# giuliojiang/pbrt-v3-IILE

Measured on AMD Instinct MI355X. Metric: Mray/s on killeroo-simple 1080p (path integrator, rays = Scene::Intersect + IntersectP calls), higher is better.
Workload: dtype f32

## Files before the change

include/iile_gpu.h:

```cpp
#ifndef IILE_GPU_H
#define IILE_GPU_H

#include "iile_scene.h"

#ifdef __cplusplus
extern "C" {
#endif

typedef struct iile_scene iile_scene;

enum {
    IILE_OK = 0,
    IILE_ERR_ARG = 1,
    IILE_ERR_NO_DEVICE = 2,
    IILE_ERR_HIP = 3,
    IILE_ERR_UNSUPPORTED = 4,
    IILE_ERR_TIMEOUT = 5
};

typedef struct iile_render_params {
    int32_t k_begin, k_end;
    int32_t tile_rank, tile_nranks;
    int32_t spp_per_pass;
    int32_t collect_stats;
    int32_t time_kernels;
    int32_t film_on_device;
    void *stream;
} iile_render_params;

typedef struct iile_stats {
    uint64_t camera_rays, closest_rays, shadow_rays;
    uint64_t nodes_closest, nodes_any, tri_tests, tri_hits;
    uint64_t sphere_tests;
    uint64_t nee_evals, zero_radiance;
    uint64_t path_length[8];
    double ms_total;
    double ms_generate, ms_extend, ms_shade, ms_connect, ms_film;
    int32_t n_extend_launches, n_connect_launches , n_shade_launches, n_passes;
    uint64_t n_paths;
    uint64_t workspace_bytes;
    uint64_t ext_rays, ext_nodes, ext_tri_tests, ext_sphere_tests;
    uint64_t any_tri_tests;
    double ms_shadow, ms_mis, ms_resolve;
    uint64_t mis_rays_traced;
    uint64_t ext_rays_traced;
} iile_stats;

int iile_device_count(void);
const char *iile_last_error(void);

int iile_device_select(int32_t device);
int iile_device_alloc(uint64_t bytes, void **out_dev);
void iile_device_free(void *dev);
int iile_device_download(void *dst_host, const void *src_dev, uint64_t bytes, void *stream);
int iile_device_upload(void *dst_dev, const void *src_host, uint64_t bytes, void *stream);
int iile_device_zero(void *dev, uint64_t bytes, void *stream);
int iile_stream_create(void **out_stream);
int iile_stream_wait(void *stream);
void iile_stream_destroy(void *stream);

int iile_scene_create(const iile_scene_desc *desc, iile_scene **out);
void iile_scene_destroy(iile_scene *scene);

int iile_render(iile_scene *scene, const iile_render_params *params, float *film_xyzw, iile_stats *stats);
int iile_render_status(iile_scene *scene, void *stream);
int iile_test_patch_capacity(iile_scene *scene, uint32_t capacity);

int iile_trace_closest(iile_scene *scene, int32_t n, const float *o3, const float *d3, const float *tmax,
                       int32_t *prim, float *tb, iile_stats *stats);
#define IILE_SHAPE_HIT_FLOATS 28
int iile_shape_hit_attributes(iile_scene *scene, int32_t n, const float *o3, const float *d3, const int32_t *prim, float *out);
int iile_trace_any(iile_scene *scene, int32_t n, const float *o3, const float *d3, const float *tmax,
                   int32_t *hit, iile_stats *stats);
int iile_halton_samples(iile_scene *scene, int32_t n, const int32_t *px, const int32_t *py, const int32_t *k,
                        int32_t dim0, int32_t ndims, float *out, uint32_t *index_out);
int iile_camera_rays(iile_scene *scene, int32_t n, const float *pfilm2, const float *plens2, float *o3, float *d3);
int iile_li_samples(iile_scene *scene, int32_t n, const int32_t *px, const int32_t *py, const int32_t *k,
                    float *L3, int32_t *nrays2);
int iile_bsdf_eval(iile_scene *scene, int32_t n, int32_t mat, const float *wo3, const float *wi3, float *out4);
int iile_bsdf_sample(iile_scene *scene, int32_t n, int32_t mat, const float *wo3, const float *u2, float *out7);
int iile_bsdf_eval_ng(iile_scene *scene, int32_t n, int32_t mat, const float *ng3, const float *wo3, const float *wi3, float *out4);
int iile_bsdf_sample_ng(iile_scene *scene, int32_t n, int32_t mat, const float *ng3, const float *wo3, const float *u2, float *out7);
int iile_bsdf_sample_specular(iile_scene *scene, int32_t n, int32_t mat, const float *wo3, const float *u2, float *out9);
int iile_render_probes(iile_scene *scene, int32_t n_probes, const float *pos3, const float *dir3, float *intensity_rgb,
                       float *normals_xyz, float *distance, int32_t outputs_on_device, iile_stats *stats, void *stream);
typedef struct iile_probe_ref_params {
    int32_t max_depth;
    int32_t first_sample;
    int32_t n_samples;
    int32_t spp_total;
    int32_t outputs_on_device;
    void *stream;
} iile_probe_ref_params;
int iile_render_probes_reference(iile_scene *scene, int32_t n_probes, const float *pos3, const float *dir3, const iile_probe_ref_params *params,
                                 float *intensity_rgb, float *weight_sum, float *normals_xyz, float *distance, iile_stats *stats);
int iile_test_probe_ref_group(iile_scene *scene, uint32_t samples_per_group);
int iile_reference_points(iile_scene *scene, int32_t n, const float *pfilm2, uint8_t *valid, float *pos3, float *dir3);
typedef struct iile_direct_params {
    int32_t n_passes, first_pass;
    int32_t accumulate;
    int32_t film_on_device;
    void *stream;
} iile_direct_params;
int iile_render_direct(iile_scene *scene, const iile_direct_params *params, double *film_rgbw);
int iile_iispt_hemi_points(iile_scene *scene, const iile_iispt_task *task, uint8_t *valid, float *pos3, float *dir3);
int iile_iispt_gather(iile_scene *scene, const iile_iispt_task *task, const uint8_t *valid, const float *pos3, const float *dir3,
                      const float *nn_films, int32_t nn_on_device, float *out_rgbw, int32_t out_on_device);
int iile_iispt_hemi_points_batch(iile_scene *scene, const iile_iispt_task *tasks, int32_t n_tasks, uint8_t *valid, float *pos3, float *dir3,
                                 void *stream);
int iile_iispt_gather_batch(iile_scene *scene, const iile_iispt_task *tasks, int32_t n_tasks, const uint8_t *valid, const float *pos3,
                            const float *dir3, const float *nn_films, int32_t nn_on_device, float *out_rgbw, int32_t out_on_device, void *stream);
int iile_iispt_film_add(iile_scene *scene, const iile_iispt_task *tasks, int32_t n_tasks, const float *out_rgbw_dev, double *film_rgbw_dev,
                        int32_t film_w, int32_t film_h, void *stream);
int iile_iispt_film_merge(const double *direct_rgbw_dev, const double *indirect_rgbw_dev, int64_t n_pixels, float *rgb_dev, void *stream);
typedef struct iile_iispt_net iile_iispt_net;
typedef struct iile_iispt_net_weights {
    const float *conv_weight[15], *conv_bias[15];
    const float *bn_weight[5], *bn_bias[5], *bn_mean[5], *bn_var[5];
    float bn_eps;
} iile_iispt_net_weights;
int iile_iispt_net_create(const iile_iispt_net_weights *weights, iile_iispt_net **out);
int iile_iispt_net_load(const char *path, iile_iispt_net **out);
int iile_iispt_net_forward(iile_iispt_net *net, const float *in_dev, float *out_dev, int32_t n, int32_t max_batch, void *stream,
                           float *layer_out_dev, int32_t layer);
int iile_iispt_net_predict(iile_iispt_net *net, const float *intensity_dev, const float *normals_dev, const float *distance_dev,
                           float *pred_dev, const int32_t *slot_of_probe_dev, int32_t n, int32_t film_rows, int32_t max_batch, void *stream);
void iile_iispt_net_destroy(iile_iispt_net *net);
typedef struct iile_bvh_build_stats {
    float ms_total, ms_morton, ms_sort, ms_treelets, ms_upper, ms_flatten, ms_download;
    int32_t n_treelets, n_nodes, n_interior, n_leaf;
} iile_bvh_build_stats;
int iile_bvh_build_hlbvh(int32_t n_prims, const float *bounds6, int32_t max_prims_in_node, iile_bvh_node *nodes_out,
                         int32_t *n_nodes_out, int32_t *order_out, iile_bvh_build_stats *stats);
int iile_bvh_pack_probe(int32_t n_nodes, const iile_bvh_node *nodes, int32_t n_interior, float *wide16, float *wide4_32,
                        int32_t *nested);
int32_t iile_wide_ref_shift(void);
void iile_traversal_limits(int32_t *out3);
int iile_light_sample_li(iile_scene *scene, int32_t light, int32_t n, const float *p3, float *out7);
int iile_light_sample_at(iile_scene *scene, int32_t light, int32_t n, const float *ref_p3, const float *ref_n3, const float *u2, float *out13);
int iile_light_pdf_at(iile_scene *scene, int32_t light, int32_t n, const float *ref_p3, const float *ref_n3, const float *wi3, float *out_pdf);
int iile_light_le(iile_scene *scene, int32_t light, int32_t n, const float *d3, float *out3);
int iile_light_choose(iile_scene *scene, int32_t n, const float *p3, const float *u, int32_t *out_light, float *out_pdf, void *stream);
int iile_texture_eval(iile_scene *scene, int32_t tex, int32_t n, const float *uv2, const float *duv4, float *rgb3);
int iile_texture_eval_p(iile_scene *scene, int32_t tex, int32_t n, const float *uv2, const float *duv4, const float *pdp9, float *rgb3);
int iile_trig_probe(int32_t n, const float *x, float *out3);

#ifdef __cplusplus
}
#endif
#endif
```

pbrt-v3-iile_amd/binding.py:

```python
import ctypes
import os

import numpy as np

_HERE = os.path.dirname(os.path.abspath(__file__))
LIB_DIR = os.path.join(_HERE, "lib")
REPO_ROOT = os.path.dirname(_HERE)
DEFAULT_SCENE = os.path.join(REPO_ROOT, "scenes", "killeroo-simple.pbrt")

c_i32, c_u32, c_u64, c_f32, c_f64 = (ctypes.c_int32, ctypes.c_uint32, ctypes.c_uint64, ctypes.c_float,
                                     ctypes.c_double)
c_vp = ctypes.c_void_p


class HostOverrides(ctypes.Structure):
    _fields_ = [("xres", c_i32), ("yres", c_i32), ("spp", c_i32), ("max_depth", c_i32), ("sampler", c_i32),
                ("accel_split", c_i32), ("bvh_build", c_vp), ("quick_render", c_i32)]


SAMPLERS = {None: 0, "": 0, "halton": 1, "sobol": 2}
SPLITS = {None: 0, "": 0, "sah": 1, "hlbvh": 2, "middle": 3, "equal": 4}


class HostSceneInfo(ctypes.Structure):
# ... 91 lines not shown


class _Sobol(ctypes.Structure):
    _fields_ = [("enabled", c_i32), ("spp", c_i32), ("resolution", c_i32), ("log2_resolution", c_i32), ("n_dims", c_i32),
                ("matrices32", c_vp), ("vdc", c_u32 * 32), ("vdc_inv", c_u32 * 32)]


class SceneDesc(ctypes.Structure):
    _fields_ = SceneDescHead._fields_ + [
        ("tri_n", c_vp), ("tri_uv", c_vp), ("prim_alpha", c_vp), ("n_spheres", c_i32), ("spheres", c_vp), ("n_materials", c_i32),
        ("materials", c_vp), ("n_lights", c_i32), ("lights", c_vp), ("n_env_dist", ctypes.c_int64), ("env_dist", c_vp),
        ("n_textures", c_i32), ("textures", c_vp), ("n_texels", ctypes.c_int64), ("texels", c_vp), ("ewa_lut", c_f32 * 128),
        ("film_filter_wide", c_i32), ("film_filter_table", c_f32 * 256), ("camera", Camera), ("film", FilmDesc), ("halton", _Halton),
        ("integrator", Integrator), ("probe", _ProbeSetup), ("sobol", _Sobol), ("n_quadrics", c_i32), ("quadrics", c_vp),
        ("light_power_all", c_vp)]


MAX_LIGHTS = 8


class Quadric(ctypes.Structure):
    _fields_ = [("o2w", c_f32 * 16), ("o2w_inv", c_f32 * 16), ("kind", c_i32), ("radius", c_f32), ("inner_radius", c_f32),
                ("height", c_f32), ("zmin", c_f32), ("zmax", c_f32), ("phi_max", c_f32), ("reverse_orientation", c_i32),
                ("swaps_handedness", c_i32)]


class Material(ctypes.Structure):
    _fields_ = [("type", c_i32), ("kd", c_f32 * 3), ("ks", c_f32 * 3), ("sigma", c_f32), ("roughness", c_f32), ("alpha", c_f32),
                ("remap_roughness", c_i32), ("eta", c_f32), ("kr", c_f32 * 3), ("kt", c_f32 * 3), ("on_a", c_f32), ("on_b", c_f32),
                ("kd_tex", c_i32), ("ks_tex", c_i32), ("kr_tex", c_i32), ("kt_tex", c_i32), ("bump_tex", c_i32), ("rough_tex", c_i32),
                ("sigma_tex", c_i32), ("opacity", c_f32 * 3), ("roughness_v", c_f32), ("alpha_v", c_f32), ("opacity_tex", c_i32),
                ("rough_tex_v", c_i32), ("cond_eta", c_f32 * 3), ("cond_k", c_f32 * 3)]


MAT_MATTE, MAT_PLASTIC, MAT_UBER, MAT_MIRROR, MAT_GLASS, MAT_METAL, MAT_SUBSTRATE = range(7)
MAT_TRANSLUCENT = 8
QUADRIC_DISK, QUADRIC_CYLINDER = 0, 1
PRIM_SPHERE, PRIM_FLIP, PRIM_QUADRIC = 1, 8, 32
LIGHT_AREA_QUADRIC = 6


class GpuStats(ctypes.Structure):
    _fields_ = [(n, c_u64) for n in ("camera_rays closest_rays shadow_rays nodes_closest nodes_any tri_tests "
                                     "tri_hits sphere_tests nee_evals zero_radiance").split()] + [
        ("path_length", c_u64 * 8),
        ("ms_total", c_f64), ("ms_generate", c_f64), ("ms_extend", c_f64), ("ms_shade", c_f64),
        ("ms_connect", c_f64), ("ms_film", c_f64),
        ("n_extend_launches", c_i32), ("n_connect_launches", c_i32), ("n_shade_launches", c_i32),
        ("n_passes", c_i32), ("n_paths", c_u64), ("workspace_bytes", c_u64),
        ("ext_rays", c_u64), ("ext_nodes", c_u64), ("ext_tri_tests", c_u64), ("ext_sphere_tests", c_u64),
        ("any_tri_tests", c_u64), ("ms_shadow", c_f64), ("ms_mis", c_f64), ("ms_resolve", c_f64),
        ("mis_rays_traced", c_u64), ("ext_rays_traced", c_u64)]

    def as_dict(self):
        d = {}
        for name, _ in self._fields_:
            v = getattr(self, name)
            d[name] = list(v) if name == "path_length" else v
        return d


HOST_SYMBOLS = ["iile_host_load_pbrt", "iile_host_scene_desc", "iile_host_scene_film", "iile_host_scene_get_info",
                "iile_host_scene_free", "iile_host_film_to_rgb", "iile_host_write_pfm", "iile_host_last_error", "iile_host_read_image",
                "iile_host_scene_texture", "iile_host_scene_texture_level", "iile_host_scene_filter_table",
                "iile_host_sobol_matrices", "iile_host_sobol_vdc", "iile_host_write_exr", "iile_host_write_image",
                "iile_host_scene_film_filename", "iile_host_scene_light", "iile_host_scene_quadric_count", "iile_host_scene_quadric",
                "iile_host_scene_material", "iile_host_scene_camera"]
class NetWeights(ctypes.Structure):
    _fields_ = [("conv_weight", c_vp * 15), ("conv_bias", c_vp * 15), ("bn_weight", c_vp * 5), ("bn_bias", c_vp * 5),
                ("bn_mean", c_vp * 5), ("bn_var", c_vp * 5), ("bn_eps", c_f32)]


class ProbeRefParams(ctypes.Structure):
    _fields_ = [("max_depth", c_i32), ("first_sample", c_i32), ("n_samples", c_i32), ("spp_total", c_i32), ("outputs_on_device", c_i32),
                ("stream", c_vp)]


class DirectParams(ctypes.Structure):
    _fields_ = [("n_passes", ctypes.c_int32), ("first_pass", ctypes.c_int32), ("accumulate", ctypes.c_int32), ("film_on_device", ctypes.c_int32),
                ("stream", ctypes.c_void_p)]


GPU_SYMBOLS = ["iile_device_count", "iile_last_error", "iile_scene_create", "iile_scene_destroy", "iile_render",
               "iile_trace_closest", "iile_trace_any", "iile_shape_hit_attributes", "iile_halton_samples", "iile_camera_rays", "iile_li_samples",
               "iile_bsdf_eval", "iile_bsdf_sample", "iile_bsdf_eval_ng", "iile_bsdf_sample_ng", "iile_bsdf_sample_specular", "iile_trig_probe", "iile_texture_eval", "iile_texture_eval_p", "iile_light_sample_li", "iile_light_sample_at", "iile_light_pdf_at", "iile_light_le", "iile_light_choose", "iile_render_probes",
               "iile_render_probes_reference", "iile_test_probe_ref_group", "iile_reference_points",
               "iile_device_select", "iile_device_alloc", "iile_device_free", "iile_device_download", "iile_device_upload", "iile_device_zero",
               "iile_stream_create", "iile_stream_wait", "iile_stream_destroy",
               "iile_iispt_film_add", "iile_iispt_film_merge",
               "iile_iispt_hemi_points", "iile_iispt_gather", "iile_iispt_hemi_points_batch", "iile_iispt_gather_batch", "iile_bvh_build_hlbvh", "iile_bvh_pack_probe", "iile_render_direct",
               "iile_wide_ref_shift", "iile_traversal_limits", "iile_render_status", "iile_test_patch_capacity", "iile_iispt_net_create", "iile_iispt_net_load", "iile_iispt_net_forward", "iile_iispt_net_predict", "iile_iispt_net_destroy"]
DIST_SYMBOLS = ["iile_dist_unique_id", "iile_dist_create", "iile_dist_create_deadline", "iile_dist_abort", "iile_dist_wait", "iile_dist_destroy", "iile_dist_rank", "iile_dist_size", "iile_dist_ranks_seen",
                "iile_dist_film_reduce", "iile_dist_monitor_reduce", "iile_dist_barrier", "iile_dist_sum_u64", "iile_dist_max_f64",
                "iile_dist_rendezvous_file", "iile_dist_rendezvous_file_token", "iile_dist_rendezvous_done", "iile_dist_all_ok",
                "iile_dist_last_error"]
DIST_ID_BYTES = 128

_host = None
_gpu = None
_dist = None


def host_lib():
    global _host
    if _host is None:
        path = os.path.join(LIB_DIR, "libiile_host.so")
        if not os.path.exists(path):
            raise RuntimeError(f"{path} is missing: run __graft_entry__.build() (make -C pbrt-v3-iile_amd/csrc host)")
        lib = ctypes.CDLL(path)
        lib.iile_host_last_error.restype = ctypes.c_char_p
        lib.iile_host_load_pbrt.argtypes = [ctypes.c_char_p, ctypes.POINTER(HostOverrides), ctypes.POINTER(c_vp)]
        lib.iile_host_scene_desc.restype = c_vp
        lib.iile_host_scene_desc.argtypes = [c_vp]
        lib.iile_host_scene_film.restype = ctypes.POINTER(FilmDesc)
        lib.iile_host_scene_film.argtypes = [c_vp]
        lib.iile_host_scene_get_info.argtypes = [c_vp, ctypes.POINTER(HostSceneInfo)]
        lib.iile_host_scene_free.argtypes = [c_vp]
        lib.iile_host_scene_free.restype = None
        lib.iile_host_scene_quadric_count.argtypes = [c_vp]
        lib.iile_host_scene_quadric_count.restype = c_i32
        lib.iile_host_scene_quadric.argtypes = [c_vp, c_i32, ctypes.POINTER(Quadric)]
        lib.iile_host_scene_material.argtypes = [c_vp, c_i32, ctypes.POINTER(Material)]
        lib.iile_host_scene_camera.argtypes = [c_vp, ctypes.POINTER(Camera)]
        lib.iile_host_film_to_rgb.argtypes = [ctypes.POINTER(FilmDesc), c_vp, c_vp]
        lib.iile_host_write_pfm.argtypes = [ctypes.c_char_p, c_vp, c_i32, c_i32]
        lib.iile_host_read_image.argtypes = [ctypes.c_char_p, ctypes.POINTER(c_i32), ctypes.POINTER(c_i32), c_vp]
        lib.iile_host_write_exr.argtypes = [ctypes.c_char_p, c_vp, c_i32, c_i32, c_i32, c_i32, c_i32, c_i32]
        lib.iile_host_write_image.argtypes = [ctypes.c_char_p, ctypes.POINTER(FilmDesc), c_vp]
        lib.iile_host_scene_film_filename.argtypes = [c_vp]
        lib.iile_host_scene_film_filename.restype = ctypes.c_char_p
        lib.iile_host_scene_texture.argtypes = [c_vp, c_i32, ctypes.POINTER(Texture)]
        lib.iile_host_scene_texture_level.argtypes = [c_vp, c_i32, c_i32, c_vp]
        lib.iile_host_scene_filter_table.argtypes = [c_vp, c_vp]
        lib.iile_host_sobol_matrices.argtypes = [c_i32, c_vp, c_vp]
        lib.iile_host_sobol_vdc.argtypes = [c_i32, c_vp, c_vp]
        _host = lib
    return _host


def sobol_matrices(n_dims):
    m32 = np.zeros((n_dims, 52), np.uint32)
    m64 = np.zeros((n_dims, 52), np.uint64)
    if host_lib().iile_host_sobol_matrices(int(n_dims), m32.ctypes.data, m64.ctypes.data) != 0:
        raise RuntimeError(host_lib().iile_host_last_error().decode())
    return m32, m64


def sobol_vdc(log2_resolution):
    vdc = np.zeros(52, np.uint64)
    inv = np.zeros(52, np.uint64)
    if host_lib().iile_host_sobol_vdc(int(log2_resolution), vdc.ctypes.data, inv.ctypes.data) != 0:
        raise RuntimeError(host_lib().iile_host_last_error().decode())
    return vdc, inv


def read_image(path):
    lib = host_lib()
    w, h = c_i32(), c_i32()
    if lib.iile_host_read_image(os.fsencode(path), ctypes.byref(w), ctypes.byref(h), None) != 0:
        raise RuntimeError(lib.iile_host_last_error().decode())
    rgb = np.empty((h.value, w.value, 3), np.float32)
    if lib.iile_host_read_image(os.fsencode(path), ctypes.byref(w), ctypes.byref(h), rgb.ctypes.data) != 0:
        raise RuntimeError(lib.iile_host_last_error().decode())
    return rgb


def write_exr(path, rgb, origin=(0, 0), display=None):
    rgb = _f32(rgb)
    h, w = rgb.shape[:2]
    x0, y0 = origin
    tw, th = display if display else (x0 + w, y0 + h)
    if host_lib().iile_host_write_exr(os.fsencode(path), rgb.ctypes.data, x0, y0, x0 + w, y0 + h, tw, th) != 0:
        raise RuntimeError(host_lib().iile_host_last_error().decode())


def gpu_lib():
    global _gpu
    if _gpu is None:
        path = os.environ.get("IILE_GPU_LIB") or os.path.join(LIB_DIR, "libiile_gpu.so")
        if not os.path.exists(path):
            raise RuntimeError(f"{path} is missing: the HIP extension was not built; there is no CPU fallback "
                               "(run __graft_entry__.build())")
        lib = ctypes.CDLL(path)
        lib.iile_last_error.restype = ctypes.c_char_p
        lib.iile_scene_create.argtypes = [c_vp, ctypes.POINTER(c_vp)]
        lib.iile_scene_destroy.argtypes = [c_vp]
        lib.iile_scene_destroy.restype = None
        lib.iile_render.argtypes = [c_vp, ctypes.POINTER(RenderParams), c_vp, ctypes.POINTER(GpuStats)]
        lib.iile_trace_closest.argtypes = [c_vp, c_i32, c_vp, c_vp, c_vp, c_vp, c_vp, ctypes.POINTER(GpuStats)]
        lib.iile_trace_any.argtypes = [c_vp, c_i32, c_vp, c_vp, c_vp, c_vp, ctypes.POINTER(GpuStats)]
        lib.iile_halton_samples.argtypes = [c_vp, c_i32, c_vp, c_vp, c_vp, c_i32, c_i32, c_vp, c_vp]
        lib.iile_camera_rays.argtypes = [c_vp, c_i32, c_vp, c_vp, c_vp, c_vp]
        lib.iile_li_samples.argtypes = [c_vp, c_i32, c_vp, c_vp, c_vp, c_vp, c_vp]
        lib.iile_bsdf_eval.argtypes = [c_vp, c_i32, c_i32, c_vp, c_vp, c_vp]
        lib.iile_texture_eval.argtypes = [c_vp, c_i32, c_i32, c_vp, c_vp, c_vp]
        lib.iile_light_sample_li.argtypes = [c_vp, c_i32, c_i32, c_vp, c_vp]
        lib.iile_light_sample_at.argtypes = [c_vp, c_i32, c_i32, c_vp, c_vp, c_vp, c_vp]
        lib.iile_light_pdf_at.argtypes = [c_vp, c_i32, c_i32, c_vp, c_vp, c_vp, c_vp]
        lib.iile_light_le.argtypes = [c_vp, c_i32, c_i32, c_vp, c_vp]
        lib.iile_light_choose.argtypes = [c_vp, c_i32, c_vp, c_vp, c_vp, c_vp, c_vp]
        lib.iile_texture_eval_p.argtypes = [c_vp, c_i32, c_i32, c_vp, c_vp, c_vp, c_vp]
        lib.iile_render_probes.argtypes = [c_vp, c_i32, c_vp, c_vp, c_vp, c_vp, c_vp, c_i32, ctypes.POINTER(GpuStats), c_vp]
        lib.iile_render_probes_reference.argtypes = [c_vp, c_i32, c_vp, c_vp, ctypes.POINTER(ProbeRefParams), c_vp, c_vp, c_vp, c_vp,
                                                     ctypes.POINTER(GpuStats)]
        lib.iile_test_probe_ref_group.argtypes = [c_vp, c_u32]
        lib.iile_reference_points.argtypes = [c_vp, c_i32, c_vp, c_vp, c_vp, c_vp]
        lib.iile_bsdf_sample.argtypes = [c_vp, c_i32, c_i32, c_vp, c_vp, c_vp]
        lib.iile_bsdf_eval_ng.argtypes = [c_vp, c_i32, c_i32, c_vp, c_vp, c_vp, c_vp]
        lib.iile_bsdf_sample_ng.argtypes = [c_vp, c_i32, c_i32, c_vp, c_vp, c_vp, c_vp]
        lib.iile_bsdf_sample_specular.argtypes = [c_vp, c_i32, c_i32, c_vp, c_vp, c_vp]
        lib.iile_trig_probe.argtypes = [c_i32, c_vp, c_vp]
        lib.iile_iispt_hemi_points.argtypes = [c_vp, ctypes.POINTER(IisptTask), c_vp, c_vp, c_vp]
        lib.iile_iispt_gather.argtypes = [c_vp, ctypes.POINTER(IisptTask), c_vp, c_vp, c_vp, c_vp, c_i32, c_vp, c_i32]
        lib.iile_iispt_hemi_points_batch.argtypes = [c_vp, ctypes.POINTER(IisptTask), c_i32, c_vp, c_vp, c_vp, c_vp]
        lib.iile_iispt_gather_batch.argtypes = [c_vp, ctypes.POINTER(IisptTask), c_i32, c_vp, c_vp, c_vp, c_vp, c_i32, c_vp, c_i32, c_vp]
        lib.iile_bvh_build_hlbvh.argtypes = [c_i32, c_vp, c_i32, c_vp, ctypes.POINTER(c_i32), c_vp, ctypes.POINTER(BvhBuildStats)]
        lib.iile_bvh_pack_probe.argtypes = [c_i32, c_vp, c_i32, c_vp, c_vp, ctypes.POINTER(c_i32)]
        lib.iile_render_status.argtypes = [c_vp, c_vp]
        lib.iile_traversal_limits.argtypes = [ctypes.POINTER(c_i32)]
        lib.iile_traversal_limits.restype = None
        lib.iile_test_patch_capacity.argtypes = [c_vp, c_u32]
        lib.iile_iispt_net_create.argtypes = [ctypes.POINTER(NetWeights), ctypes.POINTER(c_vp)]
        lib.iile_iispt_net_load.argtypes = [ctypes.c_char_p, ctypes.POINTER(c_vp)]
        lib.iile_iispt_net_forward.argtypes = [c_vp, c_vp, c_vp, c_i32, c_i32, c_vp, c_vp, c_i32]
        lib.iile_iispt_net_predict.argtypes = [c_vp, c_vp, c_vp, c_vp, c_vp, c_vp, c_i32, c_i32, c_i32, c_vp]
        lib.iile_iispt_film_add.argtypes = [c_vp, ctypes.POINTER(IisptTask), c_i32, c_vp, c_vp, c_i32, c_i32, c_vp]
        lib.iile_iispt_film_merge.argtypes = [c_vp, c_vp, ctypes.c_int64, c_vp, c_vp]
        lib.iile_device_upload.argtypes = [c_vp, c_vp, ctypes.c_uint64, c_vp]
        lib.iile_device_zero.argtypes = [c_vp, ctypes.c_uint64, c_vp]
        lib.iile_iispt_net_destroy.argtypes = [c_vp]
        lib.iile_iispt_net_destroy.restype = None
        _gpu = lib
    return _gpu


def dist_lib():
    global _dist
    if _dist is None:
        path = os.path.join(LIB_DIR, "libiile_dist.so")
        if not os.path.exists(path):
            raise RuntimeError(f"{path} is missing: run __graft_entry__.build() (make -C pbrt-v3-iile_amd/csrc dist)")
        lib = ctypes.CDLL(path)
        lib.iile_dist_last_error.restype = ctypes.c_char_p
        lib.iile_dist_unique_id.argtypes = [c_vp]
        lib.iile_dist_create.argtypes = [c_vp, c_i32, c_i32, ctypes.POINTER(c_vp)]
        lib.iile_dist_create_deadline.argtypes = [c_vp, c_i32, c_i32, ctypes.c_double, ctypes.POINTER(c_vp)]
        lib.iile_dist_wait.argtypes = [c_vp, c_vp]
        lib.iile_dist_abort.argtypes = [c_vp]
        lib.iile_dist_abort.restype = None
        lib.iile_dist_destroy.argtypes = [c_vp]
        lib.iile_dist_destroy.restype = None
        lib.iile_dist_rank.argtypes = [c_vp]
        lib.iile_dist_size.argtypes = [c_vp]
        lib.iile_dist_film_reduce.argtypes = [c_vp, c_vp, ctypes.c_int64, c_i32, c_vp]
        lib.iile_dist_barrier.argtypes = [c_vp, c_vp]
        lib.iile_dist_sum_u64.argtypes = [c_vp, c_vp, c_i32]
        lib.iile_dist_max_f64.argtypes = [c_vp, c_vp, c_i32]
        lib.iile_dist_rendezvous_file.argtypes = [ctypes.c_char_p, c_i32, c_vp, c_i32]
        lib.iile_dist_rendezvous_file_token.argtypes = [ctypes.c_char_p, c_i32, ctypes.c_uint64, c_vp, c_i32]
        lib.iile_dist_rendezvous_done.argtypes = [c_vp, ctypes.c_char_p]
        lib.iile_dist_all_ok.argtypes = [c_vp, c_i32, ctypes.POINTER(c_i32)]
        _dist = lib
    return _dist


class Dist:

    @staticmethod
    def unique_id():
        buf = (ctypes.c_uint8 * DIST_ID_BYTES)()
        lib = dist_lib()
        if lib.iile_dist_unique_id(buf) != 0:
            raise RuntimeError(f"iile_dist_unique_id failed: {lib.iile_dist_last_error().decode()}")
        return bytes(buf)

    def __init__(self, unique_id, rank, nranks, timeout_s=None):
        lib = dist_lib()
        self._c = c_vp()
        buf = (ctypes.c_uint8 * DIST_ID_BYTES).from_buffer_copy(unique_id)
        if timeout_s is None:
            rc, what = lib.iile_dist_create(buf, int(rank), int(nranks), ctypes.byref(self._c)), "iile_dist_create"
        else:
            rc, what = lib.iile_dist_create_deadline(buf, int(rank), int(nranks), float(timeout_s), ctypes.byref(self._c)), "iile_dist_create_deadline"
        if rc != 0:
            err = RuntimeError(f"{what} failed ({rc}): {lib.iile_dist_last_error().decode()}")
            err.code = rc
            raise err
        self.rank, self.size = int(rank), int(nranks)
        lib.iile_dist_ranks_seen.restype = ctypes.c_int
        lib.iile_dist_ranks_seen.argtypes = [c_vp]
        self.ranks_seen = int(lib.iile_dist_ranks_seen(self._c))

    def _check(self, rc, what):
        if rc != 0:
            raise RuntimeError(f"{what} failed ({rc}): {dist_lib().iile_dist_last_error().decode()}")

    def film_reduce(self, film_device_ptr, n_pixels, root=0, stream=None):
        self._check(dist_lib().iile_dist_film_reduce(self._c, c_vp(int(film_device_ptr)), int(n_pixels), int(root),
                                                     c_vp(stream) if stream else None), "iile_dist_film_reduce")

    def barrier(self, stream=None):
        self._check(dist_lib().iile_dist_barrier(self._c, c_vp(stream) if stream else None), "iile_dist_barrier")

    def wait(self, stream=None):
# ... 103 lines not shown
    def light_power_all(self):
        d = self.scene_desc()
        if not d.light_power_all:
            raise RuntimeError("the scene's descriptor has no light_power_all")
        return np.frombuffer(ctypes.string_at(d.light_power_all, d.n_lights * 4), dtype=np.float32).copy()

    def prim_light(self):
        head = ctypes.cast(self.desc, ctypes.POINTER(SceneDescHead)).contents
        return np.frombuffer(ctypes.string_at(head.prim_light, head.n_prims * 4), dtype=np.int32).copy()

    def camera(self):
        cam = Camera()
        kind = host_lib().iile_host_scene_camera(self._h, ctypes.byref(cam))
        if kind < 0:
            raise RuntimeError(host_lib().iile_host_last_error().decode())
        return int(kind), cam

    @property
    def quadric_count(self):
        return int(host_lib().iile_host_scene_quadric_count(self._h))

    def quadric(self, index):
        q = Quadric()
        if host_lib().iile_host_scene_quadric(self._h, int(index), ctypes.byref(q)) != 0:
            raise RuntimeError(host_lib().iile_host_last_error().decode())
        return q

    def material(self, index):
        m = Material()
        if host_lib().iile_host_scene_material(self._h, int(index), ctypes.byref(m)) != 0:
            raise RuntimeError(host_lib().iile_host_last_error().decode())
        return m

    def prim_flags(self):
        head = ctypes.cast(self.desc, ctypes.POINTER(SceneDescHead)).contents
        return np.frombuffer(ctypes.string_at(head.prim_flags, head.n_prims * 4), dtype=np.uint32).copy()

    def texture(self, index):
        lib = host_lib()
        t = Texture()
        if lib.iile_host_scene_texture(self._h, index, ctypes.byref(t)) != 0:
            raise RuntimeError(lib.iile_host_last_error().decode())
        levels = []
        for l in range(t.n_levels):
            a = np.empty((t.level_h[l], t.level_w[l], 3), np.float32)
            lib.iile_host_scene_texture_level(self._h, index, l, a.ctypes.data)
            levels.append(a)
        return t, levels

    def procedural_texture(self, index):
        t, _ = self.texture(index)
        return {"kind": t.kind, "mapping": t.mapping, "n_levels": t.n_levels, "su": t.su, "sv": t.sv, "du": t.du, "dv": t.dv,
                "vs": list(t.vs), "vt": list(t.vt), "xf": np.array(list(t.xf), np.float32).reshape(3, 4),
                "child": list(t.child), "cval": np.array([list(r) for r in t.cval], np.float32), "aamode": t.aamode,
                "bilerp": np.array([list(r) for r in t.bilerp], np.float32)}

    @property
    def film_filename(self):
        return host_lib().iile_host_scene_film_filename(self._h).decode()

    def write_image(self, path, rgb):
        rgb = _f32(rgb)
        if host_lib().iile_host_write_image(os.fsencode(path), self._film, rgb.ctypes.data) != 0:
            raise RuntimeError(host_lib().iile_host_last_error().decode())

    def write_pfm(self, path, rgb):
        rgb = _f32(rgb)
        rc = host_lib().iile_host_write_pfm(os.fsencode(path), rgb.ctypes.data, rgb.shape[1], rgb.shape[0])
        if rc != 0:
            raise RuntimeError(host_lib().iile_host_last_error().decode())

    def close(self):
        if self._h:
            host_lib().iile_host_scene_free(self._h)
            self._h = c_vp()

    def __del__(self):
        try:
            self.close()
        except Exception:
            pass


class GpuScene:

    def __init__(self, host_scene):
        lib = gpu_lib()
        self.host = host_scene
        self._s = c_vp()
        rc = lib.iile_scene_create(host_scene.desc, ctypes.byref(self._s))
        if rc != 0:
            raise RuntimeError(f"iile_scene_create failed ({rc}): {lib.iile_last_error().decode()}")

    def _check(self, rc, what):
        if rc != 0:
            raise RuntimeError(f"{what} failed ({rc}): {gpu_lib().iile_last_error().decode()}")

    def render(self, k_begin=0, k_end=0, tile_rank=0, tile_nranks=1, spp_per_pass=0, collect_stats=False,
               time_kernels=False, film_device_ptr=None, stream=None, want_stats=True):
        prm = RenderParams(int(k_begin), int(k_end), int(tile_rank), int(tile_nranks), int(spp_per_pass),
                           int(bool(collect_stats)), int(time_kernels), int(film_device_ptr is not None),
                           c_vp(stream) if stream else None)
        st = GpuStats()
        if film_device_ptr is not None:
            film, ptr = None, c_vp(int(film_device_ptr))
        else:
            h, w = self.host.film_shape
            film = np.zeros((h, w, 4), np.float32)
            ptr = film.ctypes.data
        rc = gpu_lib().iile_render(self._s, ctypes.byref(prm), ptr, ctypes.byref(st) if want_stats else None)
        self._check(rc, "iile_render")
        return film, (st.as_dict() if want_stats else None)

    def render_status(self, stream=None):
        self._check(gpu_lib().iile_render_status(self._s, c_vp(stream) if stream else None), "iile_render_status")

    def test_patch_capacity(self, capacity):
        self._check(gpu_lib().iile_test_patch_capacity(self._s, int(capacity)), "iile_test_patch_capacity")

    def trace_closest(self, o, d, tmax, instrumented=True):
        o, d, tmax = _f32(o), _f32(d), _f32(tmax)
        n = len(tmax)
        prim = np.empty(n, np.int32)
        tb = np.empty((n, 4), np.float32)
        st = GpuStats()
        self._check(gpu_lib().iile_trace_closest(self._s, n, o.ctypes.data, d.ctypes.data, tmax.ctypes.data,
                                                 prim.ctypes.data, tb.ctypes.data,
                                                 ctypes.byref(st) if instrumented else None), "iile_trace_closest")
        return prim, tb, st.as_dict()

    def shape_hit_attributes(self, o, d, prim):
        o, d, prim = _f32(o).reshape(-1, 3), _f32(d).reshape(-1, 3), _i32(prim)
        out = np.empty((len(prim), 28), np.float32)
        f = gpu_lib().iile_shape_hit_attributes
        f.argtypes = [c_vp, c_i32, c_vp, c_vp, c_vp, c_vp]
        self._check(f(self._s, len(prim), o.ctypes.data, d.ctypes.data, prim.ctypes.data, out.ctypes.data), "iile_shape_hit_attributes")
        r = {k: out[:, 3 * i:3 * i + 3] for i, k in enumerate(("p", "n", "sn", "dpdu", "dpdv", "dndu", "dndv", "wo"))}
        r.update(u=out[:, 24], v=out[:, 25], flip=out[:, 26] != 0)
        return r

    def trace_any(self, o, d, tmax, instrumented=True):
        o, d, tmax = _f32(o), _f32(d), _f32(tmax)
        n = len(tmax)
        hit = np.empty(n, np.int32)
        st = GpuStats()
        self._check(gpu_lib().iile_trace_any(self._s, n, o.ctypes.data, d.ctypes.data, tmax.ctypes.data,
                                             hit.ctypes.data, ctypes.byref(st) if instrumented else None),
                    "iile_trace_any")
        return hit, st.as_dict()

    def halton_samples(self, px, py, k, dim0, ndims):
        px, py, k = _i32(px), _i32(py), _i32(k)
        n = len(px)
        out = np.empty((n, ndims), np.float32)
        idx = np.empty(n, np.uint32)
        self._check(gpu_lib().iile_halton_samples(self._s, n, px.ctypes.data, py.ctypes.data, k.ctypes.data, dim0,
                                                  ndims, out.ctypes.data, idx.ctypes.data), "iile_halton_samples")
        return out, idx

    def camera_rays(self, pfilm, plens=None):
        pfilm = _f32(pfilm)
        n = len(pfilm)
        o = np.empty((n, 3), np.float32)
        d = np.empty((n, 3), np.float32)
        pl = _f32(plens) if plens is not None else None
        self._check(gpu_lib().iile_camera_rays(self._s, n, pfilm.ctypes.data, pl.ctypes.data if pl is not None else None,
                                               o.ctypes.data, d.ctypes.data), "iile_camera_rays")
        return o, d

    def li_samples(self, px, py, k):
        px, py, k = _i32(px), _i32(py), _i32(k)
        n = len(px)
        L = np.empty((n, 3), np.float32)
        nr = np.empty((n, 2), np.int32)
        self._check(gpu_lib().iile_li_samples(self._s, n, px.ctypes.data, py.ctypes.data, k.ctypes.data, L.ctypes.data,
                                              nr.ctypes.data), "iile_li_samples")
        return L, nr

    def bsdf_eval(self, mat, wo, wi):
        wo, wi = _f32(wo), _f32(wi)
        out = np.empty((len(wo), 4), np.float32)
        self._check(gpu_lib().iile_bsdf_eval(self._s, len(wo), mat, wo.ctypes.data, wi.ctypes.data, out.ctypes.data),
                    "iile_bsdf_eval")
        return out

    def light_sample_li(self, light, p):
        p = _f32(p).reshape(-1, 3)
        out = np.empty((len(p), 7), np.float32)
        self._check(gpu_lib().iile_light_sample_li(self._s, int(light), len(p), p.ctypes.data, out.ctypes.data), "iile_light_sample_li")
        return out

    def light_sample_at(self, light, ref_p, ref_n, u):
        ref_p, ref_n, u = _f32(ref_p).reshape(-1, 3), _f32(ref_n).reshape(-1, 3), _f32(u).reshape(-1, 2)
        assert len(ref_p) == len(ref_n) == len(u)
        out = np.empty((len(ref_p), 13), np.float32)
        self._check(gpu_lib().iile_light_sample_at(self._s, int(light), len(ref_p), ref_p.ctypes.data, ref_n.ctypes.data, u.ctypes.data,
                                                   out.ctypes.data), "iile_light_sample_at")
        return out

    def light_pdf_at(self, light, ref_p, ref_n, wi):
        ref_p, ref_n, wi = _f32(ref_p).reshape(-1, 3), _f32(ref_n).reshape(-1, 3), _f32(wi).reshape(-1, 3)
        assert len(ref_p) == len(ref_n) == len(wi)
        out = np.empty(len(ref_p), np.float32)
        self._check(gpu_lib().iile_light_pdf_at(self._s, int(light), len(ref_p), ref_p.ctypes.data, ref_n.ctypes.data, wi.ctypes.data,
                                                out.ctypes.data), "iile_light_pdf_at")
        return out

    def light_le(self, light, d):
        d = _f32(d).reshape(-1, 3)
        out = np.empty((len(d), 3), np.float32)
        self._check(gpu_lib().iile_light_le(self._s, int(light), len(d), d.ctypes.data, out.ctypes.data), "iile_light_le")
        return out

    def light_choose(self, p, u, stream=None):
        p, u = _f32(p).reshape(-1, 3), _f32(u).reshape(-1)
        light, pdf = np.empty(len(u), np.int32), np.empty(len(u), np.float32)
        self._check(gpu_lib().iile_light_choose(self._s, len(u), p.ctypes.data, u.ctypes.data, light.ctypes.data, pdf.ctypes.data,
                                                c_vp(stream) if stream else None), "iile_light_choose")
        return light, pdf

    def render_probes(self, pos, direction, hemi=None, device_out=None, stream=None):
        pos, direction = _f32(pos).reshape(-1, 3), _f32(direction).reshape(-1, 3)
        n = len(pos)
        scene_hemi = int(self.host.info["probe_hemi_size"])
        if hemi is not None and int(hemi) != scene_hemi:
            raise ValueError(f"render_probes: the scene's probe films are {scene_hemi} x {scene_hemi}, not {hemi}")
        hemi = scene_hemi
        st = GpuStats()
        if device_out is not None:
            self._check(gpu_lib().iile_render_probes(self._s, n, pos.ctypes.data, direction.ctypes.data, device_out[0], device_out[1],
                                                     device_out[2], 1, ctypes.byref(st), stream), "iile_render_probes")
            return None, None, None, st.as_dict()
        inten = np.zeros((n, hemi, hemi, 3), np.float32)
        nrm = np.zeros((n, hemi, hemi, 3), np.float32)
        dist = np.zeros((n, hemi, hemi), np.float32)
        self._check(gpu_lib().iile_render_probes(self._s, n, pos.ctypes.data, direction.ctypes.data, inten.ctypes.data,
                                                 nrm.ctypes.data, dist.ctypes.data, 0, ctypes.byref(st), stream), "iile_render_probes")
        return inten, nrm, dist, st.as_dict()

    def render_probes_reference(self, pos, direction, spp, max_depth=3, first_sample=0, spp_total=0, stream=None):
        pos, direction = _f32(pos).reshape(-1, 3), _f32(direction).reshape(-1, 3)
# ... 259 lines not shown
```

pbrt-v3-iile_amd/csrc/device/api_common.h:

```cpp
#pragma once
#include <algorithm>
#include <cstdint>
#include <string>
#include <vector>

#include "../../../include/iile_gpu.h"
#include "kernels.h"

#define HIP_TRY(expr)                                                                                        \
    do {                                                                                                     \
        hipError_t e_ = (expr);                                                                              \
        if (e_ != hipSuccess)                                                                                \
            return ::iile::api_fail(IILE_ERR_HIP, std::string(#expr) + ": " + hipGetErrorString(e_));       \
    } while (0)

namespace iile {

int ensure_device();

template <typename T>
struct DevBuf {
    T *p = nullptr;
    ~DevBuf() {
        if (p) (void)hipFree(p);
// ... 3 lines not shown
        return IILE_OK;
    }
    int put(const T *h, size_t n) {
        int rc = alloc(n);
        if (rc) return rc;
        if (n) HIP_TRY(hipMemcpy(p, h, n * sizeof(T), hipMemcpyHostToDevice));
        return IILE_OK;
    }
    int get(T *h, size_t n) {
        if (n) HIP_TRY(hipMemcpy(h, p, n * sizeof(T), hipMemcpyDeviceToHost));
        return IILE_OK;
    }
};

struct DevBlock {
    void *p = nullptr;
    size_t cap = 0;
    DevBlock() = default;
    DevBlock(const DevBlock &) = delete;
    DevBlock &operator=(const DevBlock &) = delete;
    ~DevBlock() { (void)release(); }
    bool holds(size_t bytes) const { return p && bytes <= cap; }
    hipError_t release() {
        const hipError_t e = p ? hipFree(p) : hipSuccess;
        p = nullptr;
        cap = 0;
        return e;
    }
    int reserve(size_t bytes, size_t grown = 0, const char *oom = nullptr) {
        if (holds(bytes)) return IILE_OK;
        HIP_TRY(release());
        const size_t want = std::max<size_t>(std::max(bytes, grown), 1);
        const hipError_t e = hipMalloc(&p, want);
        if (e != hipSuccess) {
            p = nullptr;
            return api_fail(IILE_ERR_HIP, oom ? std::string(oom) : "hipMalloc of a device block: " + std::string(hipGetErrorString(e)));
        }
        cap = want;
        return IILE_OK;
    }
};

struct Carver {
    char *base;
    size_t used = 0;
    explicit Carver(void *block = nullptr) : base(static_cast<char *>(block)) {}
    template <typename T>
    T *take(size_t n) {
        T *r = base ? reinterpret_cast<T *>(base + used) : nullptr;
        used += (std::max<size_t>(n, 1) * sizeof(T) + 255) & ~size_t(255);
        return r;
    }
};

struct EventPair {
    hipEvent_t a, b;
    int kind;
};

constexpr uint64_t kMaxPassPaths = 200000000ull;
static_assert(kMaxPassPaths < (uint64_t(1) << kSlotBits), "queue slots must fit kSlotBits");

}

struct iile_scene {
    iile::DScene ds;
    std::vector<void *> allocs;
    std::vector<uint8_t> prim_is_shape;
    int n_cus = 256;
    int max_depth = 5;
    int spp = 1;
    std::vector<int> light_samples;
    std::vector<int> light_types;
    uint32_t ws_paths = 0;
    iile::PassBuffers pb;
    iile::DevBlock ws_block;
    uint32_t film_tiles = 0, film_pixels = 0;
    iile::FilmBuffers fb;
    iile::DevBlock film_block, wide_block;
    uint64_t film_wide = 0;
    iile_probe_setup probe;
    const uint32_t *probe_pixel_offsets = nullptr;
    const float *probe_filter_table = nullptr;
    uint32_t *flag_count = nullptr;
    float *flag_rec = nullptr;
    iile::DevBlock probe_block;
    int *spill = nullptr;
    hipStream_t nee_stream = nullptr;
    int *spill_nee = nullptr;
    hipEvent_t ev_shade[16] = {}, ev_nee[16] = {};
    std::vector<iile::EventPair> events;
    size_t events_used = 0;
    hipEvent_t ev_begin = nullptr, ev_end = nullptr;
    std::vector<int> tile_of_slot, slot_of_tile;
    iile::DevBlock tile_tables;
    int map_key[4] = {0, 0, 0, 0};
    iile::PatchDev patch{};
    iile::DevBlock patch_block;
    iile::DevBlock film_add_block;
    uint32_t patch_cap_override = 0;
    uint32_t probe_ref_group_override = 0;
    bool overflow_unchecked = false;
    hipStream_t overflow_stream = nullptr;
    iile::DevBlock scratch;
};

namespace iile {
int ensure_workspace(iile_scene *sc, uint32_t n_paths);
int ensure_film(iile_scene *sc, uint32_t n_tiles, uint32_t n_pixels, uint64_t n_wide = 0);
int frame_pass(iile_scene *sc, const DScene &S, int rank, int nranks, hipStream_t stream, PassDesc *P);
uint64_t path_budget(double bytes_per_path);
int run_pass(iile_scene *sc, const DScene &S, int max_depth, const PassDesc &P_in, const LaunchCfg &cfg, bool timed, bool one_stream = false);
void copy_counters(const DCounters &c, iile_stats *st);
}
```

pbrt-v3-iile_amd/csrc/device/api_iispt.hip:

```cpp
#include <cmath>
#include <cstring>

#include "api_common.h"

using namespace iile;

extern "C" {
int iile_render_direct(iile_scene *sc, const iile_direct_params *prm, double *film_rgbw) {
    if (!sc || !prm || !film_rgbw || prm->n_passes < 0 || prm->first_pass < 0) return api_fail(IILE_ERR_ARG, "iile_render_direct: bad argument");
    int rc = ensure_device();
    if (rc) return rc;
    DScene S = sc->ds;
    const bool reflect_diffs = S.textured_materials && S.has_specular;
    if (S.filter_wide) return api_fail(IILE_ERR_UNSUPPORTED, "iile_render_direct: the direct pass is defined for the one-pixel box film");
    S.pb_x0 = S.samp_x0, S.pb_y0 = S.samp_y0, S.pb_x1 = S.samp_x1, S.pb_y1 = S.samp_y1, S.pb_set = 0;
    const bool tree = S.has_glass != 0;
    S.diff_scale = 0.25f;
    hipStream_t stream = static_cast<hipStream_t>(prm->stream);
    LaunchCfg cfg{sc->n_cus, stream, false};
    PassDesc P;
    rc = frame_pass(sc, S, 0, 1, stream, &P);
    if (rc) return rc;
    P.slot0 = 0;
    P.n_pass_tiles = P.n_owned_tiles;
// ... 111 lines not shown
bool invert4(const float in[16], float out[16]) {
    int indxc[4], indxr[4];
    int ipiv[4] = {0, 0, 0, 0};
    float a[4][4];
    std::memcpy(a, in, sizeof(a));
    for (int i = 0; i < 4; i++) {
        int irow = 0, icol = 0;
        float big = 0.f;
        for (int j = 0; j < 4; j++) {
            if (ipiv[j] == 1) continue;
            for (int k = 0; k < 4; k++) {
                if (ipiv[k] == 0) {
                    if (std::abs(a[j][k]) >= big) {
                        big = std::abs(a[j][k]);
                        irow = j;
                        icol = k;
                    }
                } else if (ipiv[k] > 1)
                    return false;
            }
        }
        ++ipiv[icol];
        if (irow != icol)
            for (int k = 0; k < 4; ++k) std::swap(a[irow][k], a[icol][k]);
        indxr[i] = irow;
        indxc[i] = icol;
        if (a[icol][icol] == 0.f) return false;
        const float pivinv = float(1. / double(a[icol][icol]));
        a[icol][icol] = 1.f;
        for (int j = 0; j < 4; j++) a[icol][j] *= pivinv;
        for (int j = 0; j < 4; j++) {
            if (j == icol) continue;
            const float save = a[j][icol];
            a[j][icol] = 0;
            for (int k = 0; k < 4; k++) a[j][k] -= a[icol][k] * save;
        }
    }
    for (int j = 3; j >= 0; j--)
        if (indxr[j] != indxc[j])
            for (int k = 0; k < 4; k++) std::swap(a[k][indxr[j]], a[k][indxc[j]]);
    std::memcpy(out, a, sizeof(a));
    return true;
}
struct H3 {
    float x, y, z;
};
H3 h_normalize(H3 v) {
    const float inv = 1.f / std::sqrt(v.x * v.x + v.y * v.y + v.z * v.z);
    return H3{v.x * inv, v.y * inv, v.z * inv};
}
H3 h_cross(H3 a, H3 b) {
    const double ax = a.x, ay = a.y, az = a.z, bx = b.x, by = b.y, bz = b.z;
    return H3{float((ay * bz) - (az * by)), float((az * bx) - (ax * bz)), float((ax * by) - (ay * bx))};
}
bool make_probe_camera(const float *pos, const float *dir, DProbeCam *cam) {
    const H3 up = (dir[0] == 0.0 && dir[1] == 0.0) ? H3{0.f, 1.f, 0.f} : H3{0.f, 0.f, 1.f};
    const H3 look = H3{pos[0] + dir[0], pos[1] + dir[1], pos[2] + dir[2]};
    const H3 d = h_normalize(H3{look.x - pos[0], look.y - pos[1], look.z - pos[2]});
    const H3 c = h_cross(h_normalize(up), d);
    if (std::sqrt(c.x * c.x + c.y * c.y + c.z * c.z) == 0) return false;
    const H3 right = h_normalize(c);
    const H3 new_up = h_cross(d, right);
    const float m[16] = {right.x, new_up.x, d.x, pos[0], right.y, new_up.y, d.y, pos[1], right.z, new_up.z, d.z, pos[2], 0.f, 0.f, 0.f, 1.f};
    std::memcpy(cam->c2w.m, m, sizeof(m));
    float inv[16], minv[16];
    if (!invert4(m, inv) || !invert4(inv, minv)) return false;
    for (int r = 0; r < 3; ++r)
        for (int cidx = 0; cidx < 3; ++cidx) cam->nrm[3 * r + cidx] = minv[4 * cidx + r];
    return true;
}
DScene probe_scene(const iile_scene *sc, int max_depth, float diff_scale) {
    const iile_probe_setup &pr = sc->probe;
    DScene S = sc->ds;
    const iile_film_desc &f = pr.film;
    S.probe_mode = 1;
    S.xres = f.xres, S.yres = f.yres;
    S.crop_x0 = f.crop_x0, S.crop_y0 = f.crop_y0, S.crop_x1 = f.crop_x1, S.crop_y1 = f.crop_y1;
    S.samp_x0 = f.samp_x0, S.samp_y0 = f.samp_y0, S.samp_x1 = f.samp_x1, S.samp_y1 = f.samp_y1;
    S.filter_rx = f.filter_rx, S.filter_ry = f.filter_ry;
    S.max_sample_luminance = f.max_sample_luminance;
    S.filter_wide = 1;
    S.filter_table = sc->probe_filter_table;
    S.pixel_offsets = sc->probe_pixel_offsets;
    S.base_scale0 = pr.base_scales[0], S.base_scale1 = pr.base_scales[1];
    S.base_exp0 = pr.base_exponents[0], S.base_exp1 = pr.base_exponents[1];
    S.sample_stride = pr.sample_stride;
    S.mult_inv0 = pr.mult_inverse[0], S.mult_inv1 = pr.mult_inverse[1];
    S.max_depth = max_depth;
    S.sample_center = 0;
    S.sobol = 0;
    S.lens_radius = 0;
    S.diff_scale = diff_scale;
    return S;
}
}

int iile_render_probes(iile_scene *sc, int32_t n_probes, const float *pos3, const float *dir3, float *intensity_rgb, float *normals_xyz,
                       float *distance, int32_t outputs_on_device, iile_stats *stats, void *stream_arg) {
    if (!sc || n_probes < 0 || !pos3 || !dir3 || !intensity_rgb || !normals_xyz || !distance)
        return api_fail(IILE_ERR_ARG, "iile_render_probes: null argument");
    int rc = ensure_device();
    if (rc) return rc;
    const iile_probe_setup &pr = sc->probe;
    if (pr.hemi_size <= 0 || !sc->probe_pixel_offsets) return api_fail(IILE_ERR_ARG, "iile_render_probes: the scene has no probe setup");
    if (pr.max_depth > 14) return api_fail(IILE_ERR_UNSUPPORTED, "probe maxdepth > 14");
    iile_stats st;
    std::memset(&st, 0, sizeof(st));
    if (n_probes == 0) {
        if (stats) *stats = st;
        return IILE_OK;
    }
    const DScene S = probe_scene(sc, pr.max_depth, 1.f);
    const iile_film_desc &f = pr.film;
    const int need_dims = 5 + 8 * (pr.max_depth + 1) + 2;
    if (S.n_hdims < need_dims) return api_fail(IILE_ERR_ARG, "Halton table covers too few dimensions for the probe depth");

    hipStream_t stream = static_cast<hipStream_t>(stream_arg);
    PassDesc P;
    rc = frame_pass(sc, S, 0, 1, stream, &P);
    if (rc) return rc;
    P.probe_mode = 1;
    P.probe_stx = (f.crop_x1 - f.crop_x0 + 15) / 16;
    P.probe_tiles = P.probe_stx * ((f.crop_y1 - f.crop_y0 + 15) / 16);
    P.k0 = 0;
    P.kc = 1;
    const uint32_t per_pixels = uint32_t(f.crop_x1 - f.crop_x0) * uint32_t(f.crop_y1 - f.crop_y0);
    const uint64_t slots_per_probe = uint64_t(P.probe_tiles) * 256;
    const uint64_t max_paths = path_budget(430.0);
    const int batch = int(std::max<uint64_t>(1, std::min<uint64_t>(uint64_t(n_probes), max_paths / slots_per_probe)));

    std::vector<DProbeCam> cams;
    cams.resize(size_t(n_probes));
    for (int i = 0; i < n_probes; ++i)
        if (!make_probe_camera(pos3 + 3 * size_t(i), dir3 + 3 * size_t(i), &cams[size_t(i)]))
            return api_fail(IILE_ERR_ARG, "iile_render_probes: degenerate probe direction (probe " + std::to_string(i) + ")");

    LaunchCfg cfg{sc->n_cus, stream, false};
    const uint64_t batch_paths = uint64_t(batch) * slots_per_probe;
    rc = ensure_workspace(sc, uint32_t(batch_paths));
    if (rc) return rc;
    rc = ensure_film(sc, uint32_t(uint64_t(batch) * P.probe_tiles), uint32_t(uint64_t(batch) * per_pixels), batch_paths);
    if (rc) return rc;
    DProbeCam *d_cams = nullptr;
    float *d_int = nullptr, *d_nrm = nullptr, *d_dist = nullptr;
    auto layout = [&](Carver c) {
        d_cams = c.take<DProbeCam>(size_t(batch));
        sc->pb.aux = c.take<float4>(size_t(batch_paths));
        d_int = c.take<float>(size_t(batch) * per_pixels * 3);
        d_nrm = c.take<float>(size_t(batch) * per_pixels * 3);
        d_dist = c.take<float>(size_t(batch) * per_pixels);
        return c.used;
    };
    if ((rc = sc->probe_block.reserve(layout(Carver())))) return rc;
    layout(Carver(sc->probe_block.p));
    sc->pb.nray_out = nullptr;
    sc->events_used = 0;
    HIP_TRY(hipEventRecord(sc->ev_begin, stream));
    for (int first = 0; first < n_probes; first += batch) {
        const int nb = std::min(batch, n_probes - first);
        HIP_TRY(hipMemcpyAsync(d_cams, cams.data() + first, size_t(nb) * sizeof(DProbeCam), hipMemcpyHostToDevice, stream));
        P.probe_cams = d_cams;
        P.n_owned_tiles = nb * P.probe_tiles;
        P.n_paths = uint32_t(uint64_t(nb) * slots_per_probe);
        rc = run_pass(sc, S, pr.max_depth, P, cfg, false);
        if (rc) return rc;
        const size_t px = size_t(nb) * per_pixels, off = size_t(first) * per_pixels;
// ... 448 lines not shown
```

pbrt-v3-iile_amd/csrc/device/api_probes.hip:

```cpp
#include <cstring>

#include "api_common.h"

using namespace iile;

namespace {
LaunchCfg probe_cfg(const iile_scene *sc, bool count_stats = false) { return LaunchCfg{sc->n_cus, nullptr, count_stats}; }
template <typename T>
int finish(DevBuf<T> &dev, T *host, size_t n) {
    HIP_TRY(hipGetLastError());
    HIP_TRY(hipDeviceSynchronize());
    return dev.get(host, n);
}

int trace_common(iile_scene *sc, int32_t n, const float *o3, const float *d3, const float *tmax, int any,
                 std::vector<float4> *hits, iile_stats *stats) {
    if (!sc || n < 0 || !o3 || !d3 || !tmax) return api_fail(IILE_ERR_ARG, "iile_trace: bad argument");
    int rc = ensure_device();
    if (rc) return rc;
    std::vector<float4> ro(n), rd(n);
    for (int i = 0; i < n; ++i) {
        ro[i] = make_float4(o3[3 * i], o3[3 * i + 1], o3[3 * i + 2], 0);
        rd[i] = make_float4(d3[3 * i], d3[3 * i + 1], d3[3 * i + 2], tmax[i]);
    }
// ... 1 lines not shown
    DevBuf<DCounters> dc;
    if ((rc = dro.put(ro.data(), size_t(n))) || (rc = drd.put(rd.data(), size_t(n))) || (rc = dh.alloc(2 * size_t(n))) || (rc = dc.alloc(1))) return rc;
    HIP_TRY(hipMemset(dc.p, 0, sizeof(DCounters)));
    if (n) launch_trace(sc->ds, n, dro.p, drd.p, dh.p, any, dc.p, sc->spill, probe_cfg(sc, stats != nullptr));
    hits->resize(2 * size_t(n));
    if ((rc = finish(dh, hits->data(), hits->size()))) return rc;
    if (stats) {
        DCounters c;
        if ((rc = dc.get(&c, 1))) return rc;
        std::memset(stats, 0, sizeof(*stats));
        copy_counters(c, stats);
    }
    return IILE_OK;
}

int bsdf_probe(iile_scene *sc, int32_t n, int32_t mat, const float *wo3, const float *in, size_t in_stride,
               int sample, float *out, size_t out_stride, const float *ng3 = nullptr) {
    if (!sc || n < 0 || !wo3 || !in || !out || mat < 0 || mat >= sc->ds.n_materials)
        return api_fail(IILE_ERR_ARG, "iile_bsdf: bad argument");
    const float up[3] = {0.f, 0.f, 1.f};
    if (!ng3) ng3 = up;
    int rc = ensure_device();
    if (rc) return rc;
    DevBuf<float> dwo, din, dout;
    if ((rc = dwo.put(wo3, 3 * size_t(n))) || (rc = din.put(in, in_stride * size_t(n))) ||
        (rc = dout.alloc(out_stride * size_t(n))))
        return rc;
    if (n) launch_bsdf_probe(sc->ds, n, mat, dwo.p, din.p, sample, dout.p, ng3, probe_cfg(sc));
    return finish(dout, out, out_stride * size_t(n));
}
}

extern "C" {

int iile_trace_closest(iile_scene *sc, int32_t n, const float *o3, const float *d3, const float *tmax, int32_t *prim,
                       float *tb, iile_stats *stats) {
    if (!prim || !tb) return api_fail(IILE_ERR_ARG, "iile_trace_closest: null output");
    std::vector<float4> hits;
    int rc = trace_common(sc, n, o3, d3, tmax, 0, &hits, stats);
    if (rc) return rc;
    for (int i = 0; i < n; ++i) {
        uint32_t u;
        std::memcpy(&u, &hits[2 * i].x, 4);
        prim[i] = int32_t(u);
        tb[4 * i] = hits[2 * i].y;
        tb[4 * i + 1] = hits[2 * i + 1].x;
        tb[4 * i + 2] = hits[2 * i + 1].y;
        tb[4 * i + 3] = hits[2 * i + 1].z;
    }
    return IILE_OK;
}

int iile_trace_any(iile_scene *sc, int32_t n, const float *o3, const float *d3, const float *tmax, int32_t *hit,
                   iile_stats *stats) {
    if (!hit) return api_fail(IILE_ERR_ARG, "iile_trace_any: null output");
    std::vector<float4> hits;
    int rc = trace_common(sc, n, o3, d3, tmax, 1, &hits, stats);
    if (rc) return rc;
    for (int i = 0; i < n; ++i) {
        uint32_t u;
        std::memcpy(&u, &hits[2 * i].x, 4);
        hit[i] = int32_t(u);
    }
    return IILE_OK;
}

int iile_halton_samples(iile_scene *sc, int32_t n, const int32_t *px, const int32_t *py, const int32_t *k,
                        int32_t dim0, int32_t ndims, float *out, uint32_t *index_out) {
    if (!sc || n < 0 || !px || !py || !k || !out || ndims <= 0 || dim0 < 0 || dim0 + ndims > (sc->ds.sobol ? sc->ds.sobol_dims : sc->ds.n_hdims))
        return api_fail(IILE_ERR_ARG, "iile_halton_samples: bad argument");
    int rc = ensure_device();
    if (rc) return rc;
    DevBuf<int> dx, dy, dk;
    DevBuf<float> dout;
    DevBuf<uint32_t> dindex;
    if ((rc = dx.put(px, n)) || (rc = dy.put(py, n)) || (rc = dk.put(k, n)) || (rc = dout.alloc(size_t(n) * ndims)) ||
        (rc = dindex.alloc(n)))
        return rc;
    if (n) launch_halton(sc->ds, n, dx.p, dy.p, dk.p, dim0, ndims, dout.p, dindex.p, probe_cfg(sc));
    if ((rc = finish(dout, out, size_t(n) * ndims))) return rc;
    if (index_out && (rc = dindex.get(index_out, n))) return rc;
    return IILE_OK;
}

int iile_camera_rays(iile_scene *sc, int32_t n, const float *pfilm2, const float *plens2, float *o3, float *d3) {
    if (!sc || n < 0 || !pfilm2 || !o3 || !d3) return api_fail(IILE_ERR_ARG, "iile_camera_rays: bad argument");
    int rc = ensure_device();
    if (rc) return rc;
    DevBuf<float> df, dl, dox, ddx;
    if ((rc = df.put(pfilm2, 2 * size_t(n))) || (rc = dox.alloc(3 * size_t(n))) || (rc = ddx.alloc(3 * size_t(n))))
        return rc;
    if (plens2 && (rc = dl.put(plens2, 2 * size_t(n)))) return rc;
    if (n) launch_camera(sc->ds, n, df.p, plens2 ? dl.p : nullptr, dox.p, ddx.p, probe_cfg(sc));
    if ((rc = finish(dox, o3, 3 * size_t(n))) || (rc = ddx.get(d3, 3 * size_t(n)))) return rc;
    return IILE_OK;
}

int iile_bsdf_eval(iile_scene *sc, int32_t n, int32_t mat, const float *wo3, const float *wi3, float *out4) {
    return bsdf_probe(sc, n, mat, wo3, wi3, 3, 0, out4, 4);
}
int iile_bsdf_sample(iile_scene *sc, int32_t n, int32_t mat, const float *wo3, const float *u2, float *out7) {
    return bsdf_probe(sc, n, mat, wo3, u2, 2, 1, out7, 7);
}
int iile_bsdf_eval_ng(iile_scene *sc, int32_t n, int32_t mat, const float *ng3, const float *wo3, const float *wi3, float *out4) {
    if (!ng3) return api_fail(IILE_ERR_ARG, "iile_bsdf_eval_ng: null normal");
    return bsdf_probe(sc, n, mat, wo3, wi3, 3, 0, out4, 4, ng3);
}
int iile_bsdf_sample_ng(iile_scene *sc, int32_t n, int32_t mat, const float *ng3, const float *wo3, const float *u2, float *out7) {
    if (!ng3) return api_fail(IILE_ERR_ARG, "iile_bsdf_sample_ng: null normal");
    return bsdf_probe(sc, n, mat, wo3, u2, 2, 1, out7, 7, ng3);
}

int iile_bsdf_sample_specular(iile_scene *sc, int32_t n, int32_t mat, const float *wo3, const float *u2, float *out9) {
    return bsdf_probe(sc, n, mat, wo3, u2, 2, 2, out9, 9);
}

int iile_light_sample_li(iile_scene *sc, int32_t light, int32_t n, const float *p3, float *out7) {
    if (!sc || n < 0 || !p3 || !out7 || light < 0 || light >= sc->ds.n_lights)
        return api_fail(IILE_ERR_ARG, "iile_light_sample_li: bad argument");
    if (!iile_light_is_delta(sc->light_types[size_t(light)])) return api_fail(IILE_ERR_ARG, "iile_light_sample_li: not a delta light");
    int rc = ensure_device();
    if (rc) return rc;
    DevBuf<float> dp, dout;
    if ((rc = dp.put(p3, 3 * size_t(n))) || (rc = dout.alloc(7 * size_t(n)))) return rc;
    if (n) launch_light_probe(sc->ds, n, light, dp.p, dout.p, probe_cfg(sc));
    return finish(dout, out7, 7 * size_t(n));
}

static bool light_is_sampled(int type) {
    return type == IILE_LIGHT_DIFFUSE_AREA || type == IILE_LIGHT_AREA_TRIANGLE || type == IILE_LIGHT_AREA_QUADRIC || type == IILE_LIGHT_INFINITE;
}

int iile_light_sample_at(iile_scene *sc, int32_t light, int32_t n, const float *ref_p3, const float *ref_n3, const float *u2, float *out13) {
    if (!sc || n < 0 || !ref_p3 || !ref_n3 || !u2 || !out13 || light < 0 || light >= sc->ds.n_lights)
        return api_fail(IILE_ERR_ARG, "iile_light_sample_at: bad argument");
    if (!light_is_sampled(sc->light_types[size_t(light)])) return api_fail(IILE_ERR_ARG, "iile_light_sample_at: not an area or infinite light");
    int rc = ensure_device();
    if (rc) return rc;
    DevBuf<float> dp, dn, du, dout;
    if ((rc = dp.put(ref_p3, 3 * size_t(n))) || (rc = dn.put(ref_n3, 3 * size_t(n))) || (rc = du.put(u2, 2 * size_t(n))) ||
        (rc = dout.alloc(13 * size_t(n))))
        return rc;
    if (n) launch_light_sample_probe(sc->ds, n, light, dp.p, dn.p, du.p, dout.p, probe_cfg(sc));
    return finish(dout, out13, 13 * size_t(n));
}

int iile_light_pdf_at(iile_scene *sc, int32_t light, int32_t n, const float *ref_p3, const float *ref_n3, const float *wi3, float *out_pdf) {
    if (!sc || n < 0 || !ref_p3 || !ref_n3 || !wi3 || !out_pdf || light < 0 || light >= sc->ds.n_lights)
        return api_fail(IILE_ERR_ARG, "iile_light_pdf_at: bad argument");
    if (!light_is_sampled(sc->light_types[size_t(light)])) return api_fail(IILE_ERR_ARG, "iile_light_pdf_at: not an area or infinite light");
    int rc = ensure_device();
    if (rc) return rc;
    DevBuf<float> dp, dn, dw, dout;
    if ((rc = dp.put(ref_p3, 3 * size_t(n))) || (rc = dn.put(ref_n3, 3 * size_t(n))) || (rc = dw.put(wi3, 3 * size_t(n))) ||
        (rc = dout.alloc(size_t(n))))
        return rc;
    if (n) launch_light_pdf_probe(sc->ds, n, light, dp.p, dn.p, dw.p, dout.p, probe_cfg(sc));
    return finish(dout, out_pdf, size_t(n));
}

int iile_light_le(iile_scene *sc, int32_t light, int32_t n, const float *d3, float *out3) {
    if (!sc || n < 0 || !d3 || !out3 || light < 0 || light >= sc->ds.n_lights) return api_fail(IILE_ERR_ARG, "iile_light_le: bad argument");
    if (sc->light_types[size_t(light)] != IILE_LIGHT_INFINITE) return api_fail(IILE_ERR_ARG, "iile_light_le: not an infinite light");
    int rc = ensure_device();
    if (rc) return rc;
    DevBuf<float> dd, dout;
// ... 79 lines not shown
```

pbrt-v3-iile_amd/csrc/device/api_render.hip:

```cpp
#include <chrono>
#include <cmath>
#include <cstdio>
#include <cstdlib>
#include <cstring>

#include "api_common.h"

using namespace iile;

namespace {

int get_events(iile_scene *sc, int kind, EventPair **out) {
    if (sc->events_used == sc->events.size()) {
        EventPair ep;
        HIP_TRY(hipEventCreate(&ep.a));
        HIP_TRY(hipEventCreate(&ep.b));
        sc->events.push_back(ep);
    }
    *out = &sc->events[sc->events_used++];
    (*out)->kind = kind;
    return IILE_OK;
}

template <typename Fn>
// ... 135 lines not shown
        B.counts = c.take<uint32_t>(kCntWords);
        B.counters = c.take<DCounters>(1);
        return c.used;
    };
    const size_t bytes = layout(Carver());
    const auto t_alloc = std::chrono::steady_clock::now();
    if (const int rc = sc->ws_block.reserve(bytes)) return rc;
    if (std::getenv("IILE_TIMING"))
        fprintf(stderr, "iile timing: workspace of %.1f GiB for %u paths allocated in %.3f s\n", double(bytes) / 1073741824.0, n_paths,
                std::chrono::duration<double>(std::chrono::steady_clock::now() - t_alloc).count());
    layout(Carver(sc->ws_block.p));
    B.queue_cap = uint32_t(cap);
    B.nray_out = nullptr;
    B.spill = sc->spill;
    sc->ws_paths = n_paths;
    return IILE_OK;
}

int ensure_film(iile_scene *sc, uint32_t n_tiles, uint32_t n_pixels, uint64_t n_wide) {
    if (n_wide > sc->film_wide) {
        sc->film_wide = 0;
        auto wide = [&](Carver c) {
            sc->fb.wide_L = c.take<float4>(n_wide);
            sc->fb.wide_pf = c.take<float2>(n_wide);
            return c.used;
        };
        if (const int rc = sc->wide_block.reserve(wide(Carver()), 0, "out of device memory for the sample store of a wide pixel filter (24 B per camera sample)"))
            return rc;
        wide(Carver(sc->wide_block.p));
        sc->film_wide = n_wide;
    }
    if (n_tiles <= sc->film_tiles && n_pixels <= sc->film_pixels) return IILE_OK;
    n_tiles = std::max(n_tiles, sc->film_tiles);
    n_pixels = std::max(n_pixels, sc->film_pixels);
    sc->film_tiles = sc->film_pixels = 0;
    auto film = [&](Carver c) {
        sc->fb.tile_rgbw = c.take<float4>(2 * size_t(n_tiles) * 256);
        sc->fb.film_xyzw = c.take<float4>(n_pixels);
        return c.used;
    };
    if (const int rc = sc->film_block.reserve(film(Carver()))) return rc;
    film(Carver(sc->film_block.p));
    sc->fb.k0_rgbv = sc->fb.tile_rgbw + size_t(n_tiles) * 256;
    sc->film_tiles = n_tiles;
    sc->film_pixels = n_pixels;
    return IILE_OK;
}

int frame_pass(iile_scene *sc, const DScene &S, int rank, int nranks, hipStream_t stream, PassDesc *P) {
    std::memset(P, 0, sizeof(*P));
    P->n_tiles_x = (S.samp_x1 - S.samp_x0 + 15) / 16;
    P->n_tiles_y = (S.samp_y1 - S.samp_y0 + 15) / 16;
    P->tile_rank = rank, P->tile_nranks = nranks;
    return ensure_tile_map(sc, P, stream);
}

uint64_t path_budget(double bytes_per_path) {
    double budget_mb = 65536;
    if (const char *e = std::getenv("IILE_WORKSPACE_MB")) budget_mb = std::max(64.0, atof(e));
    return std::min<uint64_t>(uint64_t(budget_mb * 1048576.0 / bytes_per_path), kMaxPassPaths);
}

void copy_counters(const DCounters &c, iile_stats *st) {
    st->camera_rays = c.camera_rays;
    st->closest_rays = c.closest_rays;
    st->shadow_rays = c.shadow_rays;
    st->nodes_closest = c.nodes_closest;
    st->nodes_any = c.nodes_any;
    st->tri_tests = c.tri_tests;
    st->tri_hits = c.tri_hits;
    st->sphere_tests = c.sphere_tests;
    st->nee_evals = c.nee_evals;
    st->zero_radiance = c.zero_radiance;
    for (int i = 0; i < 8; ++i) st->path_length[i] = c.path_length[i];
    st->ext_rays = c.ext_rays;
    st->ext_nodes = c.ext_nodes;
    st->ext_tri_tests = c.ext_tri_tests;
    st->ext_sphere_tests = c.ext_sphere_tests;
    st->any_tri_tests = c.any_tri_tests;
    st->mis_rays_traced = c.mis_traced;
    st->ext_rays_traced = c.ext_traced;
}

int run_pass(iile_scene *sc, const DScene &S, int max_depth, const PassDesc &P_in, const LaunchCfg &cfg, bool timed, bool one_stream) {
    PassBuffers &B = sc->pb;
    PassDesc P = P_in;
    P.gen_fused = !cfg.count_stats && !P.list_px && !S.has_infinite && !S.probe_mode && !B.nray_out && !S.env_camera;
    HIP_TRY(hipMemsetAsync(B.counts, 0, kCntWords * sizeof(uint32_t), cfg.stream));
    auto timed_launch_on = [&](hipStream_t stream, int kind, auto &&fn) -> int { return timed_step(sc, timed, stream, kind, fn); };
    auto timed_launch = [&](int kind, auto &&fn) -> int { return timed_launch_on(cfg.stream, kind, fn); };
    const bool two_streams = sc->nee_stream && !one_stream && !cfg.count_stats && !S.has_infinite && max_depth < 15;
    const bool nee_doubled = two_streams && !S.has_specular && B.nee_alt;
    LaunchCfg cfg_nee = cfg;
    if (two_streams) cfg_nee.stream = sc->nee_stream;
    auto buffers_of = [&](int bounce, bool nee_side) {
        PassBuffers X = B;
        if (nee_doubled && (bounce & 1)) X.nee = B.nee_alt, X.mis_hit = B.mis_hit_alt, X.nee_mis = B.nee_mis_alt;
        if (two_streams && nee_side) X.spill = sc->spill_nee;
        return X;
    };
    int rc = IILE_OK;
    if (P.gen_fused) {
        HIP_TRY(hipMemsetD32Async(reinterpret_cast<hipDeviceptr_t>(&B.counts[0]), int(P.n_paths), 1, cfg.stream));
    } else {
        rc = timed_launch(0, [&] { launch_generate(S, P, B, cfg); });
        if (rc) return rc;
    }
    P.skip_last_bounce = 0;
    if (!cfg.count_stats && max_depth >= 1 && !S.probe_mode && !B.nray_out)
        P.skip_last_bounce = S.has_specular ? 1 : 2;
    const int last_bounce = (P.skip_last_bounce == 2) ? max_depth - 1 : max_depth;
    for (int b = 0; b <= last_bounce; ++b) {
        rc = timed_launch(1, [&] { launch_extend(S, P, B, b, B.queue_cap, cfg); });
        if (rc) return rc;
        if (S.has_infinite) {
            rc = timed_launch(6, [&] { launch_miss(S, B, b, B.queue_cap, cfg); });
            if (rc) return rc;
        }
        if (two_streams && !nee_doubled && b > 0) HIP_TRY(hipStreamWaitEvent(cfg.stream, sc->ev_nee[b - 1], 0));
        if (nee_doubled && b > 1) HIP_TRY(hipStreamWaitEvent(cfg.stream, sc->ev_nee[b - 2], 0));
        const PassBuffers B_shade = buffers_of(b, false), B_nee = buffers_of(b, true);
        rc = timed_launch(2, [&] { launch_shade(S, P, B_shade, b, B.queue_cap, cfg); });
        if (rc) return rc;
        if (b < max_depth) {
            if (two_streams) {
                HIP_TRY(hipEventRecord(sc->ev_shade[b], cfg.stream));
                HIP_TRY(hipStreamWaitEvent(cfg_nee.stream, sc->ev_shade[b], 0));
            }
            rc = timed_launch_on(cfg_nee.stream, 5, [&] { launch_mis(S, B_nee, b, B.queue_cap, cfg_nee); });
            if (rc) return rc;
            rc = timed_launch_on(cfg_nee.stream, 6, [&] { launch_mis_lit(S, B_nee, b, B.queue_cap, cfg_nee); });
            if (rc) return rc;
            rc = timed_launch_on(cfg_nee.stream, 3, [&] { launch_shadow(S, B_nee, b, B.queue_cap, cfg_nee); });
            if (rc) return rc;
            if (two_streams) HIP_TRY(hipEventRecord(sc->ev_nee[b], cfg_nee.stream));
        }
    }
    if (two_streams && max_depth > 0) HIP_TRY(hipStreamWaitEvent(cfg.stream, sc->ev_nee[max_depth - 1], 0));
    HIP_TRY(hipGetLastError());
    return IILE_OK;
}
}

extern "C" {
int iile_render(iile_scene *sc, const iile_render_params *prm, float *film_xyzw, iile_stats *stats) {
    if (!sc || !prm || !film_xyzw) return api_fail(IILE_ERR_ARG, "iile_render: null argument");
    int rc = ensure_device();
    if (rc) return rc;
    rc = check_pending_overflow(sc);
    if (rc) return rc;
    const DScene &S = sc->ds;
    int k_begin = prm->k_begin, k_end = prm->k_end;
    if (k_end <= 0) {
        k_begin = 0;
        k_end = sc->spp;
    }
    if (k_begin < 0 || k_begin >= k_end) return api_fail(IILE_ERR_ARG, "iile_render: empty sample range");
    int rank = prm->tile_rank, nranks = prm->tile_nranks;
    if (nranks <= 0) {
        rank = 0;
        nranks = 1;
    }
    if (rank < 0 || rank >= nranks) return api_fail(IILE_ERR_ARG, "iile_render: tile_rank out of range");
    hipStream_t stream = static_cast<hipStream_t>(prm->stream);
    LaunchCfg cfg{sc->n_cus, stream, prm->collect_stats != 0};
    const bool timed = prm->time_kernels != 0;

    PassDesc P;
    rc = frame_pass(sc, S, rank, nranks, stream, &P);
// ... 179 lines not shown
```

pbrt-v3-iile_amd/csrc/device/api_scene.hip:

```cpp
#include <array>
#include <cmath>
#include <cstring>
#include <limits>
#include <map>

#include "api_common.h"

using namespace iile;

namespace {
thread_local std::string g_err;
}
namespace iile {
int api_fail(int code, const std::string &msg) {
    g_err = msg;
    return code;
}
int ensure_device() {
    int n = 0;
    hipError_t e = hipGetDeviceCount(&n);
    if (e != hipSuccess || n <= 0)
        return api_fail(IILE_ERR_NO_DEVICE,
                        "no HIP device available: libiile_gpu has no CPU fallback (hipGetDeviceCount: " +
                            std::string(e == hipSuccess ? "0 devices" : hipGetErrorString(e)) + ")");
    return IILE_OK;
}
int check_bvh_nodes(const iile_bvh_node *nodes, int n_nodes, int64_t max_prims, const char *prefix, int *n_interior) {
    *n_interior = 0;
    for (int i = 0; i < n_nodes; ++i) {
        const iile_bvh_node &nd = nodes[i];
        if (nd.nprims > 0) {
            if (nd.offset < 0 || nd.offset + int64_t(nd.nprims) > max_prims) return api_fail(IILE_ERR_ARG, std::string(prefix) + "bad leaf range");
            continue;
        }
        if (i + 1 >= n_nodes || nd.offset <= i || nd.offset >= n_nodes) return api_fail(IILE_ERR_ARG, std::string(prefix) + "bad BVH child index");
        ++*n_interior;
    }
    return IILE_OK;
}
}
namespace {

template <typename T>
int upload(iile_scene *sc, const T *host, size_t n, const T **dev) {
    void *p = nullptr;
    size_t bytes = std::max<size_t>(n, 1) * sizeof(T);
    HIP_TRY(hipMalloc(&p, bytes));
    sc->allocs.push_back(p);
    if (n) HIP_TRY(hipMemcpy(p, host, n * sizeof(T), hipMemcpyHostToDevice));
    *dev = static_cast<const T *>(p);
    return IILE_OK;
}

DMaterial device_material(const iile_material &m, int n_textures) {
    DMaterial r = DMaterial();
    r.type = m.type;
    for (int c = 0; c < 3; ++c) {
        r.kd[c] = m.kd[c];
        r.ks[c] = m.ks[c];
        r.kr[c] = m.kr[c];
        r.kt[c] = m.kt[c];
        r.cond_eta[c] = m.type == IILE_MAT_METAL ? m.cond_eta[c] : 0.f;
        r.cond_k[c] = m.type == IILE_MAT_METAL ? m.cond_k[c] : 0.f;
        r.opacity[c] = m.type == IILE_MAT_UBER ? m.opacity[c] : 1.f;
    }
    r.alpha = m.alpha;
    const bool uv_rough = m.type == IILE_MAT_METAL || m.type == IILE_MAT_SUBSTRATE;
    r.alpha_y = (m.type == IILE_MAT_GLASS || uv_rough) ? m.alpha_v : (m.type == IILE_MAT_UBER && m.rough_tex_v != -2) ? m.alpha_v : m.alpha;
    const bool oren_nayar = m.type == IILE_MAT_MATTE && m.sigma != 0;
    r.on_a = oren_nayar ? m.on_a : 1.f;
    r.on_b = oren_nayar ? m.on_b : 0.f;
    r.eta = m.eta;
    const bool tex = n_textures > 0;
    r.kd_tex = tex ? m.kd_tex : -1, r.ks_tex = tex ? m.ks_tex : -1, r.kr_tex = tex ? m.kr_tex : -1, r.kt_tex = tex ? m.kt_tex : -1;
    r.opacity_tex = (tex && m.type == IILE_MAT_UBER) ? m.opacity_tex : -1;
    r.rough_tex_v = (m.type == IILE_MAT_UBER || uv_rough) ? ((m.rough_tex_v >= 0 && !tex) ? -1 : m.rough_tex_v) : -2;
    r.bump_tex = tex ? m.bump_tex : -1, r.rough_tex = tex ? m.rough_tex : -1, r.sigma_tex = tex ? m.sigma_tex : -1;
    r.remap_roughness = m.remap_roughness;
    return r;
}
std::array<int, 9> material_textures(const DMaterial &m) {
    return {m.kd_tex, m.ks_tex, m.kr_tex, m.kt_tex, m.bump_tex, m.rough_tex, m.sigma_tex, m.opacity_tex, m.rough_tex_v};
}
int texture_input(const iile_texture &t, int k) { return t.kind == IILE_TEX_IMAGE ? -1 : t.child[k]; }
// ... 519 lines not shown
    S.samp_x0 = f.samp_x0, S.samp_y0 = f.samp_y0, S.samp_x1 = f.samp_x1, S.samp_y1 = f.samp_y1;
    const int32_t *pb = d.integrator.pixel_bounds;
    const bool given = pb[0] != 0 || pb[1] != 0 || pb[2] != 0 || pb[3] != 0;
    S.pb_x0 = given ? std::max(pb[0], f.samp_x0) : f.samp_x0, S.pb_y0 = given ? std::max(pb[1], f.samp_y0) : f.samp_y0;
    S.pb_x1 = given ? std::min(pb[2], f.samp_x1) : f.samp_x1, S.pb_y1 = given ? std::min(pb[3], f.samp_y1) : f.samp_y1;
    S.pb_set = (S.pb_x0 != f.samp_x0 || S.pb_y0 != f.samp_y0 || S.pb_x1 != f.samp_x1 || S.pb_y1 != f.samp_y1) ? 1 : 0;
    S.filter_rx = f.filter_rx, S.filter_ry = f.filter_ry, S.max_sample_luminance = f.max_sample_luminance;
    S.max_depth = d.integrator.max_depth, S.rr_threshold = d.integrator.rr_threshold;
    sc->max_depth = d.integrator.max_depth;
    return IILE_OK;
}

int build_runtime(iile_scene *sc, const iile_scene_desc &) {
    int rc = scene_alloc(sc, size_t(max_traversal_threads(sc->n_cus)) * sizeof(int), &sc->spill, "hipMalloc(spill) failed");
    if (!rc) rc = scene_alloc(sc, size_t(max_traversal_threads(sc->n_cus)) * sizeof(int), &sc->spill_nee, "hipMalloc(spill) failed");
    if (!rc) rc = scene_alloc(sc, 256 + size_t(kMaxFlagged) * 6 * sizeof(float), &sc->flag_count, "hipMalloc(flag records) failed");
    if (rc) return rc;
    sc->flag_rec = reinterpret_cast<float *>(reinterpret_cast<char *>(sc->flag_count) + 256);
    if (hipStreamCreateWithFlags(&sc->nee_stream, hipStreamNonBlocking) != hipSuccess) return api_fail(IILE_ERR_HIP, "hipStreamCreate failed");
    for (int i = 0; i < 16; ++i)
        if (hipEventCreateWithFlags(&sc->ev_shade[i], hipEventDisableTiming) != hipSuccess ||
            hipEventCreateWithFlags(&sc->ev_nee[i], hipEventDisableTiming) != hipSuccess)
            return api_fail(IILE_ERR_HIP, "hipEventCreate failed");
    if (hipEventCreate(&sc->ev_begin) != hipSuccess || hipEventCreate(&sc->ev_end) != hipSuccess) return api_fail(IILE_ERR_HIP, "hipEventCreate failed");
    return IILE_OK;
}

int build_light_distribution(iile_scene *sc, const iile_scene_desc &d) {
    DScene &S = sc->ds;
    S.light_nv[0] = S.light_nv[1] = S.light_nv[2] = 1;
    const int n = d.n_lights;
    const size_t stride = light_record_floats(n);
    if (n > 1 && d.integrator.light_strategy != IILE_LIGHTS_SPATIAL) {
        std::vector<float> tab(stride, 0.f);
        const float *power = n > IILE_MAX_LIGHTS ? d.light_power_all : d.integrator.light_power;
        float *func = tab.data(), *cdf = tab.data() + n;
        for (int i = 0; i < n; ++i) func[i] = d.integrator.light_strategy == IILE_LIGHTS_UNIFORM ? 1.f : power[i];
        cdf[0] = 0;
        for (int i = 1; i < n + 1; ++i) cdf[i] = cdf[i - 1] + func[i - 1] / n;
        const float func_int = cdf[n];
        if (func_int == 0)
            for (int i = 1; i < n + 1; ++i) cdf[i] = float(i) / float(n);
        else
            for (int i = 1; i < n + 1; ++i) cdf[i] /= func_int;
        tab[2 * size_t(n) + 1] = func_int;
        return upload(sc, tab.data(), tab.size(), &S.light_dist);
    }
    if (!spatial_table(d)) return IILE_OK;
    light_grid(d, S.light_nv);
    std::vector<float> samples(128 * 5);
    const int bases[5] = {2, 3, 5, 7, 11};
    for (int i = 0; i < 128; ++i)
        for (int b = 0; b < 5; ++b) {
            if (b == 0) {
                uint64_t v = uint64_t(i), r = 0;
                for (int k = 0; k < 64; ++k) r |= ((v >> k) & 1ull) << (63 - k);
                samples[5 * i] = float(double(r) * 0x1p-64);
                continue;
            }
            const float inv_base = 1.f / float(bases[b]);
            uint64_t a = uint64_t(i), rev = 0;
            float inv_base_n = 1;
            while (a) {
                const uint64_t next = a / uint64_t(bases[b]);
                rev = rev * uint64_t(bases[b]) + (a - next * uint64_t(bases[b]));
                inv_base_n *= inv_base;
                a = next;
            }
            samples[5 * i + b] = std::min(float(rev) * inv_base_n, 0x1.fffffep-1f);
        }
    const float *dsamples = nullptr;
    float *dist = nullptr;
    const size_t n_vox = size_t(S.light_nv[0]) * S.light_nv[1] * S.light_nv[2];
    int rc = upload(sc, samples.data(), samples.size(), &dsamples);
    if (!rc) rc = scene_alloc(sc, n_vox * stride * sizeof(float), &dist, "hipMalloc(light distributions) failed");
    if (rc) return rc;
    S.light_dist = dist;
    LaunchCfg cfg{sc->n_cus, nullptr, false};
    launch_light_distributions(S, dsamples, dist, cfg);
    if (hipDeviceSynchronize() != hipSuccess || hipGetLastError() != hipSuccess) return api_fail(IILE_ERR_HIP, "light distribution kernel failed");
    return IILE_OK;
}

}

extern "C" {

const char *iile_last_error(void) { return g_err.c_str(); }

int iile_device_count(void) {
    int n = 0;
    if (hipGetDeviceCount(&n) != hipSuccess) return 0;
    return n;
}

int iile_device_select(int32_t device) {
    int rc = ensure_device();
    if (rc) return rc;
    HIP_TRY(hipSetDevice(device));
    return IILE_OK;
}
int iile_device_alloc(uint64_t bytes, void **out_dev) {
    if (!out_dev) return api_fail(IILE_ERR_ARG, "iile_device_alloc: null argument");
    int rc = ensure_device();
    if (rc) return rc;
    HIP_TRY(hipMalloc(out_dev, std::max<size_t>(size_t(bytes), 1)));
    return IILE_OK;
}
void iile_device_free(void *dev) {
    if (dev) (void)hipFree(dev);
}
int iile_device_download(void *dst_host, const void *src_dev, uint64_t bytes, void *stream) {
    if (!dst_host || !src_dev) return api_fail(IILE_ERR_ARG, "iile_device_download: null argument");
    hipStream_t s = static_cast<hipStream_t>(stream);
    HIP_TRY(hipMemcpyAsync(dst_host, src_dev, size_t(bytes), hipMemcpyDeviceToHost, s));
    HIP_TRY(hipStreamSynchronize(s));
    return IILE_OK;
}

int iile_device_upload(void *dst_dev, const void *src_host, uint64_t bytes, void *stream) {
    if (!dst_dev || !src_host) return api_fail(IILE_ERR_ARG, "iile_device_upload: null argument");
    hipStream_t s = static_cast<hipStream_t>(stream);
    HIP_TRY(hipMemcpyAsync(dst_dev, src_host, size_t(bytes), hipMemcpyHostToDevice, s));
    HIP_TRY(hipStreamSynchronize(s));
    return IILE_OK;
}
int iile_stream_create(void **out_stream) {
    if (!out_stream) return api_fail(IILE_ERR_ARG, "iile_stream_create: null argument");
    int rc = ensure_device();
    if (rc) return rc;
    hipStream_t s = nullptr;
    HIP_TRY(hipStreamCreateWithFlags(&s, hipStreamNonBlocking));
    *out_stream = s;
    return IILE_OK;
}
int iile_stream_wait(void *stream) {
    HIP_TRY(hipStreamSynchronize(static_cast<hipStream_t>(stream)));
    return IILE_OK;
}
void iile_stream_destroy(void *stream) {
    if (stream) (void)hipStreamDestroy(static_cast<hipStream_t>(stream));
}
int iile_device_zero(void *dev, uint64_t bytes, void *stream) {
    if (!dev) return api_fail(IILE_ERR_ARG, "iile_device_zero: null argument");
    HIP_TRY(hipMemsetAsync(dev, 0, size_t(bytes), static_cast<hipStream_t>(stream)));
    return IILE_OK;
}

static_assert(kLightDiffuseArea == IILE_LIGHT_DIFFUSE_AREA && kLightPoint == IILE_LIGHT_POINT &&
                  kLightSpot == IILE_LIGHT_SPOT && kLightDistant == IILE_LIGHT_DISTANT &&
                  kLightAreaTriangle == IILE_LIGHT_AREA_TRIANGLE && kLightInfinite == IILE_LIGHT_INFINITE &&
                  kLightAreaQuadric == IILE_LIGHT_AREA_QUADRIC && kLightProjection == IILE_LIGHT_PROJECTION &&
                  kLightGoniometric == IILE_LIGHT_GONIOMETRIC,
              "light type codes");
static_assert(kQuadricDisk == IILE_QUADRIC_DISK && kQuadricCylinder == IILE_QUADRIC_CYLINDER && kMaxQuadrics == IILE_MAX_QUADRICS,
              "quadric kind codes");
static_assert(kMatMatte == IILE_MAT_MATTE && kMatPlastic == IILE_MAT_PLASTIC && kMatUber == IILE_MAT_UBER &&
                  kMatMirror == IILE_MAT_MIRROR && kMatGlass == IILE_MAT_GLASS && kMatMetal == IILE_MAT_METAL &&
                  kMatSubstrate == IILE_MAT_SUBSTRATE && kMatTranslucent == IILE_MAT_TRANSLUCENT,
              "material type codes");
static_assert(kShapeHitFloats == IILE_SHAPE_HIT_FLOATS, "shape hit record");
static_assert(kTexImage == IILE_TEX_IMAGE && kTexScale == IILE_TEX_SCALE && kTexMix == IILE_TEX_MIX && kTexChecker2D == IILE_TEX_CHECKER2D &&
                  kTexChecker3D == IILE_TEX_CHECKER3D && kTexUV == IILE_TEX_UV && kTexBilerp == IILE_TEX_BILERP && kMapUV == IILE_MAP_UV &&
                  kMapSpherical == IILE_MAP_SPHERICAL && kMapCylindrical == IILE_MAP_CYLINDRICAL && kMapPlanar == IILE_MAP_PLANAR &&
                  kAAClosedForm == IILE_AA_CLOSEDFORM && kAANone == IILE_AA_NONE,
              "texture kinds");
int iile_scene_create(const iile_scene_desc *d, iile_scene **out) {
    if (!d || !out) return api_fail(IILE_ERR_ARG, "iile_scene_create: null argument");
    int rc = check_scene_desc(*d);
    if (!rc) rc = ensure_device();
    if (rc) return rc;
    iile_scene *sc = new iile_scene;
    std::memset(&sc->ds, 0, sizeof(sc->ds));
    std::memset(&sc->pb, 0, sizeof(sc->pb));
    std::memset(&sc->fb, 0, sizeof(sc->fb));
    hipDeviceProp_t prop;
    int dev = 0;
    if (hipGetDevice(&dev) == hipSuccess && hipGetDeviceProperties(&prop, dev) == hipSuccess)
        sc->n_cus = prop.multiProcessorCount;
    set_kernel_flags(*d, sc->ds);
    for (auto build : {build_bvh, build_top4, build_prims, build_shapes, build_materials, build_textures, build_lights, build_halton,
                       build_sobol, build_camera_film, build_runtime, build_light_distribution}) {
        rc = build(sc, *d);
        if (rc) {
            iile_scene_destroy(sc);
            return rc;
        }
    }
    *out = sc;
    return IILE_OK;
}

void iile_scene_destroy(iile_scene *sc) {
    if (!sc) return;
    for (void *p : sc->allocs) (void)hipFree(p);
    if (sc->nee_stream) (void)hipStreamDestroy(sc->nee_stream);
    for (int i = 0; i < 16; ++i) {
        if (sc->ev_shade[i]) (void)hipEventDestroy(sc->ev_shade[i]);
        if (sc->ev_nee[i]) (void)hipEventDestroy(sc->ev_nee[i]);
    }
    for (EventPair &e : sc->events) {
        (void)hipEventDestroy(e.a);
        (void)hipEventDestroy(e.b);
    }
    if (sc->ev_begin) (void)hipEventDestroy(sc->ev_begin);
    if (sc->ev_end) (void)hipEventDestroy(sc->ev_end);
    delete sc;
}
}
```

pbrt-v3-iile_amd/csrc/device/dpath.h:

```cpp
#pragma once
#include "dscene.h"

namespace iile {

DEV uint32_t div_magic(uint32_t a, uint32_t magic, uint32_t shift) {
    uint32_t t = __umulhi(magic, a);
    return (t + ((a - t) >> 1)) >> shift;
}

DEV uint32_t halton_index(const DScene &S, int px, int py, uint32_t k) {
    int pmx = px - (px / 128) * 128, pmy = py - (py / 128) * 128;
    if (pmx < 0) pmx += 128;
    if (pmy < 0) pmy += 128;
    return S.pixel_offsets[pmy * 128 + pmx] + k * uint32_t(S.sample_stride);
}

DEV float radical_inverse_base2(uint32_t a) {
    unsigned long long rev = (unsigned long long)__brev(a) << 32;
    return float(double(rev) * 0x1p-64);
}
DEV float radical_inverse_base3(uint32_t a0) {
    const float inv_base = 1.f / 3.f;
    double a = double(a0), reversed = 0;
    float inv_base_n = 1;
// ... 47 lines not shown
        if (!all) break;
        uint32_t digit[N], p[N];
#pragma unroll
        for (int i = 0; i < N; ++i) {
            const double next = __builtin_trunc(__builtin_fma(a[i], hd[i].inv_base_d, 0.5 * hd[i].inv_base_d));
            digit[i] = uint32_t(__builtin_fma(-next, hd[i].base_d, a[i]));
            a[i] = next;
        }
#pragma unroll
        for (int i = 0; i < N; ++i) p[i] = uint32_t(perms[hd[i].perm_offset + digit[i]]);
#pragma unroll
        for (int i = 0; i < N; ++i) {
            reversed[i] = __builtin_fma(reversed[i], hd[i].base_d, double(p[i]));
            inv_base_n[i] *= hd[i].inv_base;
        }
    }
#pragma unroll
    for (int i = 0; i < N; ++i) {
        while (a[i] != 0) {
            const double next = __builtin_trunc(__builtin_fma(a[i], hd[i].inv_base_d, 0.5 * hd[i].inv_base_d));
            const uint32_t digit = uint32_t(__builtin_fma(-next, hd[i].base_d, a[i]));
            reversed[i] = __builtin_fma(reversed[i], hd[i].base_d, double(uint32_t(perms[hd[i].perm_offset + digit])));
            inv_base_n[i] *= hd[i].inv_base;
            a[i] = next;
        }
    }
#pragma unroll
    for (int i = 0; i < N; ++i)
        out[i] = mn(inv_base_n[i] * (float(reversed[i]) + hd[i].perm0_term), kOneMinusEpsilon);
}
DEV uint32_t sobol_xor4(const uint32_t *bt, uint32_t w) {
    return bt[w & 255u] ^ bt[256u + ((w >> 8) & 255u)] ^ bt[512u + ((w >> 16) & 255u)] ^ bt[768u + (w >> 24)];
}
DEV uint32_t sobol_index(const DScene &S, int px, int py, uint32_t k) {
    const int m = S.sobol_log2res, m2 = 2 * m;
    const uint32_t delta = sobol_xor4(S.sobol_vdc_bt, k);
    const uint32_t b = ((uint32_t(px - S.samp_x0) << m) | uint32_t(py - S.samp_y0)) ^ delta;
    return (k << m2) ^ sobol_xor4(S.sobol_vdc_bt + 1024, b);
}
template <typename PermPtr>
DEV float sobol_sample_dimension(const DScene &S, PermPtr mats, uint32_t index, int dim, int px, int py) {
    (void)mats;
    const uint32_t v = sobol_xor4(S.sobol_bt + size_t(dim) * 1024, index);
    float s = mn(float(v) * 0x1p-32f , kOneMinusEpsilon);
    if (dim == 0 || dim == 1) {
        const int pmin = dim == 0 ? S.samp_x0 : S.samp_y0, cur = dim == 0 ? px : py;
        s = s * float(S.sobol_res) + float(pmin);
        s = s - float(cur);
        s = s < 0.f ? 0.f : (s > kOneMinusEpsilon ? kOneMinusEpsilon : s);
    }
    return s;
}

DEV uint32_t sample_index(const DScene &S, int px, int py, uint32_t k) {
    return S.sobol ? sobol_index(S, px, py, k) : halton_index(S, px, py, k);
}
template <typename PermPtr>
DEV float sample_dimension(const DScene &S, PermPtr perms, uint32_t index, int dim, int px = 0, int py = 0) {
    if (S.sobol) return sobol_sample_dimension(S, perms, index, dim, px, py);
    if (S.sample_center && dim < 2) return 0.5f;
    if (dim == 0) return radical_inverse_base2(index >> S.base_exp0);
    if (dim == 1) return radical_inverse_base3(index / uint32_t(S.base_scale1));
    return scrambled_radical_inverse(S, perms, dim, index);
}
template <typename PermPtr>
DEV float sample_dimension_hi(const DScene &S, PermPtr perms, uint32_t index, int dim) {
    if (dim < 2) __builtin_unreachable();
    return sample_dimension(S, perms, index, dim);
}
DEV float sample_dimension(const DScene &S, uint32_t index, int dim, int px = 0, int py = 0) {
    return sample_dimension(S, S.perms, index, dim, px, py);
}
template <int N, typename PermPtr>
DEV void sample_dimensions_n(const DScene &S, PermPtr perms, int dim0, bool dim_uniform, int dim_lane, uint32_t index, float *out) {
    if (dim_lane < 2) __builtin_unreachable();
    if (S.sobol) {
#pragma unroll
        for (int i = 0; i < N; ++i) out[i] = sobol_sample_dimension(S, perms, index, dim_lane + i, 0, 0);
    } else if (dim_uniform) {
        scrambled_radical_inverse_n<N>(S, perms, dim0, index, out);
    } else {
        for (int i = 0; i < N; ++i) out[i] = sample_dimension_hi(S, perms, index, dim_lane + i);
    }
}

DEV void concentric_sample_disk(float u0, float u1, float *dx, float *dy) {
    float ox = 2.f * u0 - 1, oy = 2.f * u1 - 1;
    if (ox == 0 && oy == 0) {
        *dx = 0;
        *dy = 0;
        return;
    }
    float theta, r;
    if (fabsf(ox) > fabsf(oy)) {
        r = ox;
        theta = kPiOver4 * (oy / ox);
    } else {
        r = oy;
        theta = kPiOver2 - kPiOver4 * (ox / oy);
    }
    float s, c;
    sincos_f(theta, &s, &c);
    *dx = r * c;
    *dy = r * s;
}
DEV F3 cosine_sample_hemisphere(float u0, float u1) {
    float dx, dy;
    concentric_sample_disk(u0, u1, &dx, &dy);
    float z = sqrtf(mx(0.f, 1 - dx * dx - dy * dy));
    return F3{dx, dy, z};
}

DEV float opaque_zero() {
    float z = 0.f;
    asm volatile("" : "+v"(z));
    return z;
}
static __device__ __attribute__((noinline)) F3 env_camera_direction(float pfx, float pfy, int xres, int yres) {
    const float theta = kPi * pfy / float(yres);
    const float phi = 2 * kPi * pfx / float(xres);
    float st, ct, sp, cp;
    sincos_f(theta, &st, &ct);
    sincos_f(phi, &sp, &cp);
    return F3{st * cp, ct, st * sp};
}
template <bool ANY_CAMERA = true>
DEV void camera_ray(const DScene &S, float pfx, float pfy, float lu0, float lu1, F3 *o_out, F3 *d_out, float *tmax,
                    const float zero = 0.f) {
    F3 ro = F3{zero, zero, zero};
    F3 rd;
    if (ANY_CAMERA && S.env_camera) {
        rd = env_camera_direction(pfx, pfy, S.xres, S.yres);
    } else {
        F3 pcam = xf_point(S.raster_to_camera, F3{pfx, pfy, zero});
        rd = normalize(pcam);
        if (S.lens_radius > 0) {
            float lx, ly;
            concentric_sample_disk(lu0, lu1, &lx, &ly);
            lx = S.lens_radius * lx;
            ly = S.lens_radius * ly;
            float ft = S.focal_distance / rd.z;
            F3 pfocus = ro + rd * ft;
            ro = F3{lx, ly, zero};
            rd = normalize(pfocus - ro);
        }
    }
    F3 oerr;
    F3 o = xf_point_err(S.camera_to_world, ro, &oerr);
    F3 d = xf_vector(S.camera_to_world, rd);
    float len2 = length_sq(d);
    float tm = IILE_INF;
    if (len2 > 0) {
        float dt = dot(vabs(d), oerr) / len2;
        o = o + d * dt;
        tm -= dt;
    }
    *o_out = o;
    *d_out = d;
    *tmax = tm;
}

DEV void probe_ray(const DScene &S, const DProbeCam &cam, float pfx, float pfy, F3 *o_out, F3 *d_out, float *tmax) {
    const float theta = kPi * pfy / float(S.yres);
    const float phi = kPi * pfx / float(S.xres);
    float st, ct, sp, cp;
    sincos_f(theta, &st, &ct);
// ... 626 lines not shown
```

pbrt-v3-iile_amd/csrc/device/dscene.h:

```cpp
#pragma once
#include "../../../include/iile_scene.h"
#include "dmath.h"

namespace iile {

struct DSphere {
    M44 o2w, o2w_inv;
    float radius, zmin, zmax, theta_min, theta_max, phi_max;
    int reverse_orientation, swaps_handedness;
    float center[3];
    float pad_;
};
enum { kQuadricDisk = 0, kQuadricCylinder = 1 };
struct DQuadric {
    M44 o2w, o2w_inv;
    int kind;
    float radius, inner_radius, height, zmin, zmax, phi_max;
    int reverse_orientation, swaps_handedness;
};
enum { kMatMatte = 0, kMatPlastic = 1, kMatUber = 2, kMatMirror = 3, kMatGlass = 4, kMatMetal = 5, kMatSubstrate = 6,
       kMatTranslucent = 8 };
struct alignas(16) DMaterial {
    int type;
    float kd[3];
// ... 49 lines not shown
    int quadric;
};
struct DHaltonDim {
    uint32_t base, perm_offset;
    float inv_base;
    float perm0_term;
    double base_d;
    double inv_base_d;
};
constexpr int kMaxHaltonDims = 128;
constexpr int kMaxSpheres = 8;
constexpr int kMaxQuadrics = 1024;
constexpr int kMaxMaterials = 64;
constexpr uint32_t light_record_floats(int n_lights) { return 2u * uint32_t(n_lights) + 2u; }

struct DProbeCam {
    M44 c2w;
    float nrm[9];
};

#ifndef IILE_TOP_RECORDS
#define IILE_TOP_RECORDS 21
#endif
constexpr int kMaxTop = IILE_TOP_RECORDS;
constexpr int kRefShift = 2;
constexpr int kTopFlag = 1 << 28;

struct DScene {
    const float4 *wide;
    const float4 *wide4;
    const float4 *tri_verts;
    const float4 *tri_norms;
    const float2 *tri_uv;
    const int *prim_shape;
    const int2 *prim_alpha;
    const uint16_t *perms;
    const DHaltonDim *hdims;
    const uint32_t *pixel_offsets;
    const DSphere *spheres;
    const DQuadric *quadrics;
    const DMaterial *materials;
    const DLight *lights;
    const DTexture *textures;
    const float4 *texels;
    const float *ewa_lut;
    const float *env_dist;
    int n_textures;
    int textured_materials;
    int n_nodes, n_prims, n_spheres, n_materials, n_lights, n_hdims;
    int n_quadrics;
    int n_perms;
    float root_box[6];
    int root_ref;
    const float4 *top4;
    int n_top;
    int root_ref_top;
    const float *light_dist;
    int light_nv[3];
    int has_infinite;
    int extended_features;
    int all_lights_infinite;
    int has_glass;
    int has_uber_trans;
    int has_specular;
    int has_alpha;
    int rare_prims;
    int boxes_nested;
    M44 raster_to_camera, camera_to_world;
    float lens_radius, focal_distance;
    float dx_camera[3], dy_camera[3];
    int env_camera;
    float diff_scale;
    int xres, yres;
    int crop_x0, crop_y0, crop_x1, crop_y1;
    int samp_x0, samp_y0, samp_x1, samp_y1;
    int pb_x0, pb_y0, pb_x1, pb_y1;
    int pb_set;
    float filter_rx, filter_ry, max_sample_luminance;
    int probe_mode;
    int filter_wide;
    const float *filter_table;
    int base_scale0, base_scale1, base_exp0, base_exp1, sample_stride, mult_inv0, mult_inv1;
    int sample_center;
    int sobol, sobol_log2res, sobol_res, sobol_dims;
    const uint32_t *sobol_mat;
    const uint32_t *sobol_vdc;
    const uint32_t *sobol_bt;
    const uint32_t *sobol_vdc_bt;
    int max_depth;
    float rr_threshold;
};

enum { NEE_HAS_SHADOW = 1, NEE_HAS_MIS = 2 };

struct DCounters {
    unsigned long long camera_rays, closest_rays, shadow_rays;
    unsigned long long nodes_closest, nodes_any, tri_tests, tri_hits, sphere_tests;
    unsigned long long nee_evals, zero_radiance;
    unsigned long long path_length[8];
    unsigned long long ext_rays, ext_nodes, ext_tri_tests, ext_sphere_tests;
    unsigned long long any_tri_tests;
    unsigned long long mis_traced;
    unsigned long long ext_traced;
};

}
```

pbrt-v3-iile_amd/csrc/device/kernels.h:

```cpp
#pragma once
#include <string>

#include "../../../include/iile_scene.h"
#include "dscene.h"

namespace iile {

struct PassDesc {
    int n_tiles_x, n_tiles_y, tile_rank, tile_nranks, n_owned_tiles;
    const int *tile_of_slot, *slot_of_tile;
    int slot0, n_pass_tiles;
    int k0, kc;
    uint32_t n_paths;
    const int *list_px, *list_py, *list_k;
    int probe_mode, probe_tiles, probe_stx;
    const DProbeCam *probe_cams;
    int gen_fused;
    int skip_last_bounce;
    uint32_t direct_seed;
    int direct_arrays;
    const unsigned long long *direct_jump;
    const int *direct_nsamples;
    int direct_total_samples;
    int direct_levels;
};

constexpr int kSlotBits = 28;
constexpr int kCntWords = 128;
struct PassBuffers {
    uint32_t queue_cap;
    float4 *L;
    float4 *beta;
    uint32_t *hindex;
    float *eta_scale;
    float4 *ray_o[2];
    float4 *ray_d[2];
    float4 *ray_s[2];
    float4 *hits;
    float4 *mis_hit;
    float4 *nee_alt, *mis_hit_alt;
    uint8_t *nee_mis_alt;
    float4 *nee;
    uint8_t *nee_mis;
    uint32_t *shade_q;
    uint32_t *counts;
    DCounters *counters;
    uint32_t *nray_out;
    int *spill;
    float4 *aux;
    uint32_t *flag_count;
    float *flag_rec;
    float4 *dir_E, *dir_F;
    float4 *dir_RD;
    uint32_t dir_paths;
};
constexpr uint32_t kMaxFlagged = 1u << 20;

struct FilmBuffers {
    float4 *tile_rgbw;
    float4 *k0_rgbv;
    float4 *film_xyzw;
    float4 *wide_L;
    float2 *wide_pf;
};

struct PatchDev {
    uint32_t *counters;
    uint4 *hits;
    uint32_t *keys;
    uint32_t *heads;
    uint32_t table_mask;
    uint4 *ent_a;
    float4 *ent_b;
    uint32_t cap_hits, cap_entries;
};
constexpr uint32_t kPatchNil = 0xffffffffu;

struct LaunchCfg {
    int n_cus;
    hipStream_t stream;
    bool count_stats;
    int trav_blocks_per_cu = 0;
};

int api_fail(int code, const std::string &msg);
int check_bvh_nodes(const iile_bvh_node *nodes, int n_nodes, int64_t max_prims, const char *prefix, int *n_interior);
int pack_wide_records(const iile_bvh_node *d_nodes, int n_nodes, int n_interior, float4 *d_wide, float4 *d_wide4, int *nested_out,
                      const int *d_remap = nullptr);

uint32_t queue_capacity(uint32_t n_paths, int n_cus);
void launch_generate(const DScene &S, const PassDesc &P, const PassBuffers &B, const LaunchCfg &cfg);
void launch_extend(const DScene &S, const PassDesc &P, const PassBuffers &B, int bounce, uint32_t max_rays, const LaunchCfg &cfg);
void launch_shade(const DScene &S, const PassDesc &P, const PassBuffers &B, int bounce, uint32_t max_rays, const LaunchCfg &cfg);
void launch_shadow(const DScene &S, const PassBuffers &B, int bounce, uint32_t max_rays, const LaunchCfg &cfg);
void launch_mis(const DScene &S, const PassBuffers &B, int bounce, uint32_t max_rays, const LaunchCfg &cfg);
void launch_light_distributions(const DScene &S, const float *samples, float *out, const LaunchCfg &cfg);
void launch_miss(const DScene &S, const PassBuffers &B, int bounce, uint32_t max_rays, const LaunchCfg &cfg);
void launch_mis_lit(const DScene &S, const PassBuffers &B, int bounce, uint32_t max_rays, const LaunchCfg &cfg);
void launch_film_accumulate(const DScene &S, const PassDesc &P, const PassBuffers &B, const FilmBuffers &F,
                            const LaunchCfg &cfg);
void launch_film_store(const DScene &S, const PassDesc &P, const PassBuffers &B, const FilmBuffers &F, int k_begin, int n_samples,
                       const LaunchCfg &cfg);
void launch_film_gather(const DScene &S, const PassDesc &P, const FilmBuffers &F, int n_samples, const LaunchCfg &cfg);
bool launch_probe_film(const DScene &S, const PassDesc &P, const PassBuffers &B, int n_probes, float *intensity, float *normals, float *distance,
                       const LaunchCfg &cfg);
int probe_film_tiles(const DScene &S);
void launch_probe_film_add(const DScene &S, const PassDesc &P, const PassBuffers &B, int n_probes, float4 *acc, int n_ord, float *normals, float *distance,
                           const LaunchCfg &cfg);
void launch_probe_film_resolve(const DScene &S, const PassDesc &P, int n_probes, float4 *acc, int n_ord, float *intensity, float *weight_sum, const LaunchCfg &cfg);
void launch_direct_generate(const DScene &S, const PassDesc &P, const PassBuffers &B, const LaunchCfg &cfg);
void launch_direct_shade(const DScene &S, const PassDesc &P, const PassBuffers &B, int depth, uint32_t max_rays, const LaunchCfg &cfg);
void launch_direct_tree(const DScene &S, const PassDesc &P, const PassBuffers &B, double *film_rgbw, const LaunchCfg &cfg);
void launch_direct_miss(const DScene &S, const PassBuffers &B, int depth, uint32_t max_rays, const LaunchCfg &cfg);
void launch_direct_fold(const DScene &S, const PassDesc &P, const PassBuffers &B, double *film_rgbw, const LaunchCfg &cfg);
void launch_probe_finish(const DScene &S, const PassDesc &P, const PassBuffers &B, const FilmBuffers &F, int n_probes,
                         float *intensity, float *normals, float *distance, const LaunchCfg &cfg);
void launch_film_resolve(const DScene &S, const PassDesc &P, const FilmBuffers &F, const LaunchCfg &cfg);

struct DHemiCam {
    M44 c2w;
    float w2c[9];
    float look[3], origin[3];
    int valid;
};
struct IisptItems {
    float4 *ro, *rd, *beta, *hit, *pf;
    uint32_t *idx;
    uint32_t *n_active;
    int n_items, n_hemi, nx;
};
struct IisptJob {
    iile_iispt_task T;
    IisptItems I;
    int ny;
    uint8_t *valid;
    float *pos3, *dir3;
    const DHemiCam *cams;
    const float *nn_films;
    float4 *out;
};
int launch_iispt_first_hits(const DScene &S, const IisptJob *jobs, int n_jobs, int max_items, uint32_t *n_active, int *spill, const LaunchCfg &cfg);
void launch_iispt_hemi_out(const DScene &S, const IisptJob *jobs, int n_jobs, int max_hemi, const LaunchCfg &cfg);
void launch_reference_rays(const DScene &S, int n, const float *pfilm2, float4 *ro, float4 *rd, const LaunchCfg &cfg);
void launch_reference_points(const DScene &S, int n, const float4 *ro, const float4 *rd, const float4 *hits, uint8_t *valid, float *pos3, float *dir3,
                             const LaunchCfg &cfg);
void launch_iispt_gather(const DScene &S, const IisptJob *jobs, int n_jobs, int max_pixels, const float *jac, const LaunchCfg &cfg);
void launch_iispt_film_add(const int4 *rects, const uint32_t *first, int n_tasks, int max_pixels, const float4 *out, double *film, int film_w, hipStream_t stream);
void launch_iispt_film_merge(const double *a, const double *b, float *rgb, long long n, hipStream_t stream);

void launch_trace(const DScene &S, int n, const float4 *ro, const float4 *rd, float4 *hits, int any_hit,
                  DCounters *counters, int *spill, const LaunchCfg &cfg);
uint32_t max_traversal_threads(int n_cus);
struct TraversalLimits {
    int lds_stack, top_records, max_bvh_depth;
};
TraversalLimits traversal_limits();
int default_trav_blocks_per_cu();
void launch_halton(const DScene &S, int n, const int *px, const int *py, const int *k, int dim0, int ndims,
                   float *out, uint32_t *index_out, const LaunchCfg &cfg);
void launch_camera(const DScene &S, int n, const float *pfilm, const float *plens, float *o, float *d,
                   const LaunchCfg &cfg);
void launch_bsdf_probe(const DScene &S, int n, int mat, const float *wo, const float *wi_or_u, int sample,
                       float *out, const float ng[3], const LaunchCfg &cfg);
void launch_trig_probe(int n, const float *x, float *out, const LaunchCfg &cfg);
void launch_patch_pass(const DScene &S, const PassDesc &P, const PassBuffers &B, const FilmBuffers &F, const PatchDev &D, const LaunchCfg &cfg);
void launch_patch_merge(const DScene &S, const PassDesc &P, const FilmBuffers &F, const PatchDev &D, const LaunchCfg &cfg);
void launch_light_probe(const DScene &S, int n, int light, const float *p, float *out, const LaunchCfg &cfg);
void launch_light_sample_probe(const DScene &S, int n, int light, const float *p, const float *nrm, const float *u, float *out, const LaunchCfg &cfg);
void launch_light_pdf_probe(const DScene &S, int n, int light, const float *p, const float *nrm, const float *w, float *out, const LaunchCfg &cfg);
void launch_light_le_probe(const DScene &S, int n, int light, const float *d, float *out, const LaunchCfg &cfg);
void launch_light_choose(const DScene &S, int n, const float *p, const float *u, int *light, float *pdf, const LaunchCfg &cfg);
void launch_texture_probe(const DScene &S, int n, int tex, const float *uv, const float *duv, const float *pdp, float *out,
                          const LaunchCfg &cfg);
constexpr int kShapeHitFloats = 28;
void launch_shape_hit_probe(const DScene &S, int n, const float *o, const float *d, const int *prim, float *out, const LaunchCfg &cfg);

}
```

pbrt-v3-iile_amd/csrc/device/kernels.hip:

```cpp
#include "kcommon.h"

namespace iile {

__global__ __launch_bounds__(kBlock) void k_generate(DScene S, PassDesc P, PassBuffers B, int count_stats) {
    unsigned long long n_cam = 0;
    for (uint32_t base = blockIdx.x * kBlock; base < P.n_paths; base += gridDim.x * kBlock) {
        const uint32_t pid = base + threadIdx.x;
        bool valid = pid < P.n_paths;
        int px = 0, py = 0;
        uint32_t k = 0;
        if (valid) valid = path_pixel(S, P, pid, &px, &py, &k);
        F3 o = F3{0, 0, 0}, d = F3{0, 0, 1};
        float tmax = 0;
        if (valid) {
            const uint32_t idx = sample_index(S, px, py, k);
            const float u0 = sample_dimension(S, idx, 0, px, py), u1 = sample_dimension(S, idx, 1, px, py);
            float l0 = 0, l1 = 0;
            if (S.lens_radius > 0) {
                l0 = sample_dimension(S, idx, 3);
                l1 = sample_dimension(S, idx, 4);
            }
            if (P.probe_mode) {
                const uint32_t probe = (pid / uint32_t(P.kc)) / (256u * uint32_t(P.probe_tiles));
                probe_ray(S, P.probe_cams[probe], float(px) + u0, float(py) + u1, &o, &d, &tmax);
                B.aux[pid] = make_float4(0, 0, 0, -1.f);
            } else
                camera_ray(S, float(px) + u0, float(py) + u1, l0, l1, &o, &d, &tmax);
            if (!P.list_px && !P.probe_mode) flag_whole_film_position(B, pid, px, py, k, float(px) + u0, float(py) + u1, u0, u1);
            B.hindex[pid] = idx;
            B.L[pid] = make_float4(0, 0, 0, 0);
            if (B.nray_out) {
                B.nray_out[2 * pid] = 0;
                B.nray_out[2 * pid + 1] = 0;
            }
            ++n_cam;
        } else if (pid < P.n_paths) {
            B.L[pid] = make_float4(0, 0, 0, 0);
        }
        if (pid < P.n_paths) {
            B.ray_o[0][pid] = make_float4(o.x, o.y, o.z, b2f(valid ? pid : kInvalid));
            B.ray_d[0][pid] = make_float4(d.x, d.y, d.z, tmax);
        }
    }
    if (blockIdx.x == 0 && threadIdx.x == 0) B.counts[kCntRay] = P.n_paths;
    if (count_stats) flush_counter(&B.counters->camera_rays, n_cam);
}

__global__ __launch_bounds__(kBlock) void k_miss(DScene S, PassBuffers B, int bounce) {
    const uint32_t count = B.counts[kCntRay + bounce];
    const float4 *ro = B.ray_o[bounce & 1], *rd = B.ray_d[bounce & 1];
    for (uint32_t slot = blockIdx.x * kBlock + threadIdx.x; slot < count; slot += gridDim.x * kBlock) {
        const float4 h4 = B.hits[slot];
        if (int(f2b(h4.x)) >= 0) continue;
        const uint32_t pid = f2b(ro[slot].w);
        if (pid == kInvalid) continue;
        const float4 d4 = rd[slot];
        const float4 beta4 = bounce == 0 ? make_float4(1, 1, 1, b2f(5u)) : B.ray_s[bounce & 1][slot];
        const uint32_t state_w = bounce == 0 ? 5u : f2b(d4.w);
        if (!((bounce == 0 && !S.probe_mode) || (bounce != 0 && (state_w >> 16) != 0))) continue;
        const F3 beta = F3{beta4.x, beta4.y, beta4.z}, d = F3{d4.x, d4.y, d4.z};
        const float4 L4 = B.L[pid];
        F3 L = F3{L4.x, L4.y, L4.z};
        for (int l = 0; l < S.n_lights; ++l)
            if (S.lights[l].type == kLightInfinite) L = L + beta * inf_le(S, S.lights[l], d);
        B.L[pid] = make_float4(L.x, L.y, L.z, 0);
    }
}

__global__ __launch_bounds__(kBlock) void k_mis_lit(DScene S, PassBuffers B, int bounce, uint32_t plane) {
    const uint32_t count = B.counts[kCntMis + bounce];
    for (uint32_t q = blockIdx.x * kBlock + threadIdx.x; q < count; q += gridDim.x * kBlock) {
        const float4 n2 = B.nee[2 * size_t(plane) + q];
        const uint32_t e = f2b(n2.w);
        if (e == kInvalid) continue;
        const uint32_t mis = B.nee_mis[e];
        if (mis == 0) continue;
        const float4 n3 = B.nee[3 * size_t(plane) + q];
        const int li = int(f2b(n3.w));
        bool lit = false;
        if (mis == 255u) {
            lit = S.lights[li].type == kLightInfinite;
        } else {
            const float4 h4 = B.mis_hit[e];
            const int prim = int(f2b(h4.x));
            if (int(f2b(S.tri_verts[3 * size_t(prim) + 2].w)) == li)
                lit = mis_ray_lit(S, li, prim, h4.y, h4.z, h4.w, F3{n2.x, n2.y, n2.z}, F3{n3.x, n3.y, n3.z});
        }
        B.nee_mis[e] = lit ? 1 : 0;
    }
}

DEV F3 guard_radiance(const DScene &S, F3 L) {
    const float y = lum_y(L);
    if (is_nan(L.x) || is_nan(L.y) || is_nan(L.z))
        L = F3{0, 0, 0};
    else if (double(y) < -1e-5)
        L = F3{0, 0, 0};
    else if (is_inf(y))
        L = F3{0, 0, 0};
    const float y2 = lum_y(L);
    if (y2 > S.max_sample_luminance) L = L * (S.max_sample_luminance / y2);
    return L;
}
// ... 894 lines not shown
```

pbrt-v3-iile_amd/csrc/device/kernels_shade.hip:

```cpp
#include <cstdlib>

#include "kcommon.h"

namespace iile {

DEV F3 sample_li_plain(const DScene &S, const DLight &lt, F3 po, float u0, float u1, float *pdf) {
    *pdf = 1;
    if (lt.type == kLightInfinite) {
        F3 wi, target;
        return inf_sample_li(S, lt, po, u0, u1, &wi, pdf, &target);
    }
    if (iile_light_is_delta(lt.type)) {
        F3 wi, target;
        return delta_light_li(S, lt, po, &wi, &target);
    }
    Isect ref;
    ref.p = po;
    ref.perr = F3{0, 0, 0};
    ref.n = F3{0, 0, 0};
    const LightSample ps = shape_sample(S, lt, ref, u0, u1, pdf);
    if (*pdf == 0 || length_sq(ps.p - po) == 0) {
        *pdf = 0;
        return F3{0, 0, 0};
    }
    const F3 wi = normalize(ps.p - po);
    return area_light_L(lt, ps.n, -wi);
}
DEV float lerp_f(float t, float a, float b) { return (1 - t) * a + t * b; }
__global__ __launch_bounds__(128) void k_light_contrib(DScene S, const float *samples, float *out, uint32_t stride) {
    const int nv0 = S.light_nv[0], nv1 = S.light_nv[1], nv2 = S.light_nv[2];
    const int v = blockIdx.x * blockDim.x + threadIdx.x, j = blockIdx.y;
    if (v >= nv0 * nv1 * nv2 || j >= S.n_lights) return;
    const int pi2 = v % nv2, pi1 = (v / nv2) % nv1, pi0 = v / (nv2 * nv1);
    const F3 bmin = F3{S.root_box[0], S.root_box[1], S.root_box[2]}, bmax = F3{S.root_box[3], S.root_box[4], S.root_box[5]};
    const F3 p0 = F3{float(pi0) / float(nv0), float(pi1) / float(nv1), float(pi2) / float(nv2)};
    const F3 p1 = F3{float(pi0 + 1) / float(nv0), float(pi1 + 1) / float(nv1), float(pi2 + 1) / float(nv2)};
    const F3 vmin = F3{lerp_f(p0.x, bmin.x, bmax.x), lerp_f(p0.y, bmin.y, bmax.y), lerp_f(p0.z, bmin.z, bmax.z)};
    const F3 vmax = F3{lerp_f(p1.x, bmin.x, bmax.x), lerp_f(p1.y, bmin.y, bmax.y), lerp_f(p1.z, bmin.z, bmax.z)};
    const DLight &lt = S.lights[j];
    float contrib = 0;
    for (int i = 0; i < 128; ++i) {
        const float *t = samples + 5 * i;
        const F3 po = F3{lerp_f(t[0], vmin.x, vmax.x), lerp_f(t[1], vmin.y, vmax.y), lerp_f(t[2], vmin.z, vmax.z)};
        float pdf;
        const F3 Li = sample_li_plain(S, lt, po, t[3], t[4], &pdf);
        if (pdf > 0) contrib += lum_y(Li) / pdf;
    }
    out[size_t(v) * stride + size_t(j)] = contrib;
}
__global__ __launch_bounds__(128) void k_light_cdf(DScene S, float *out) {
    const int v = blockIdx.x * blockDim.x + threadIdx.x;
    if (v >= S.light_nv[0] * S.light_nv[1] * S.light_nv[2]) return;
    const int n = S.n_lights;
    float *d = out + size_t(v) * light_record_floats(n);
    float sum = 0;
    for (int j = 0; j < n; ++j) sum = sum + d[j];
    const float avg = sum / float(128 * n);
    const float min_contrib = (avg > 0) ? float(.001 * double(avg)) : 1.f;
    float cdf = 0;
    d[n] = 0;
    for (int j = 0; j < n; ++j) {
        const float f = mx(d[j], min_contrib);
        d[j] = f;
        cdf = cdf + f / float(n);
        d[n + 1 + j] = cdf;
    }
    const float func_int = cdf;
    d[2 * n + 1] = func_int;
    for (int i = 1; i < n + 1; ++i) {
        if (func_int == 0)
            d[n + i] = float(i) / float(n);
        else
            d[n + i] = d[n + i] / func_int;
    }
}

#ifndef IILE_SHADE_WAVES
#define IILE_SHADE_WAVES 4
#endif
#ifndef IILE_SHADE_WAVES_TEX
#define IILE_SHADE_WAVES_TEX 3
#endif
constexpr int shade_waves(bool tex) { return tex ? IILE_SHADE_WAVES_TEX : IILE_SHADE_WAVES; }
template <bool COUNT, bool EXT, bool TEX>
__global__ __launch_bounds__(kBlock, shade_waves(TEX)) void k_shade(DScene S, PassDesc P, PassBuffers B, int bounce, uint32_t plane) {
    extern __shared__ __attribute__((aligned(16))) uint16_t s_perms_raw[];
    if (S.sobol) {
    } else {
        for (int i = threadIdx.x; i < S.n_perms; i += kBlock) s_perms_raw[i] = S.perms[i];
    }
    __syncthreads();
    lds_u16 *const s_perms = (lds_u16 *)s_perms_raw;
    const uint32_t count = B.counts[kCntShade + bounce];
    const float4 *ro = B.ray_o[bounce & 1], *rd = B.ray_d[bounce & 1];
    float4 *no = B.ray_o[(bounce + 1) & 1], *nd = B.ray_d[(bounce + 1) & 1];
    const float4 *rs = B.ray_s[bounce & 1];
    float4 *ns = B.ray_s[(bounce + 1) & 1];
    unsigned long long n_nee = 0, n_term = 0, n_pdf_tests = 0, n_pdf_hits = 0;
    DiagSums<IILE_SWITCH(IILE_SHADE_STAMPS) && !COUNT, 8> stamps;
    WaveOut ray_out{0, 0}, nee_out{0, 0}, mis_out{0, 0};
    auto pad_ray = [&](uint32_t sl) { no[sl] = make_float4(0, 0, 0, b2f(kInvalid)); };
    auto pad_nee = [&](uint32_t sl) { B.nee[plane + sl] = B.nee[4 * plane + sl] = make_float4(0, 0, 0, b2f(kInvalid)); };
    auto pad_mis = [&](uint32_t sl) { B.nee[2 * plane + sl] = make_float4(0, 0, 0, b2f(kInvalid)); };
    __shared__ uint32_t s_entry[kWavesPerBlock][kShadeChunk];
    const int lane = threadIdx.x & 63, wave = threadIdx.x >> 6;
    uint32_t *const head = &B.counts[kCntShdHead + bounce];
    for (;;) {
        uint32_t base = 0;
        if (lane == 0) base = atomicAdd(head, uint32_t(kShadeChunk));
        base = __builtin_amdgcn_readfirstlane(base);
        if (base >= count) break;
        uint32_t ent[kShadeChunk / 64];
#pragma unroll
        for (int j = 0; j < kShadeChunk / 64; ++j) {
            const uint32_t qi = base + uint32_t(j) * 64u + uint32_t(lane);
            ent[j] = qi < count ? B.shade_q[qi] : kInvalid;
        }
        uint32_t run = 0;
        for (uint32_t c = 0; c < 8; ++c) {
#pragma unroll
            for (int j = 0; j < kShadeChunk / 64; ++j) {
                const bool is_c = (ent[j] == kInvalid ? 7u : ent[j] >> kSlotBits) == c;
                const uint64_t m = __ballot(is_c);
                if (is_c)
                    s_entry[wave][run + __builtin_amdgcn_mbcnt_hi(uint32_t(m >> 32), __builtin_amdgcn_mbcnt_lo(uint32_t(m), 0u))] = ent[j];
                run += uint32_t(__popcll(m));
            }
        }
        __builtin_amdgcn_fence(__ATOMIC_ACQ_REL, "wavefront");
        __builtin_amdgcn_wave_barrier();
        stamps.mark(0);
      for (int round = 0; round < kShadeChunk / 64; ++round) {
        const uint32_t mine = s_entry[wave][round * 64 + lane];
        const bool valid = mine != kInvalid;
        if (__ballot(valid) == 0) break;
        const uint32_t slot = mine & ((1u << kSlotBits) - 1u);
        bool surface = false;
        bool alive = false, returned_early = false;
        uint32_t pid = 0, hidx = 0;
        int dim = 0;
        Isect is;
        Bsdf bsdf;
        F3 beta = F3{0, 0, 0}, ray_d = F3{0, 0, 1};
        uint32_t state_next = 0;
        {
            bool emit_nee = false;
            F3 so = F3{0, 0, 0}, sd = F3{0, 0, 1}, mo = F3{0, 0, 0}, md = F3{0, 0, 1};
            F3 A = F3{0, 0, 0}, Bc = F3{0, 0, 0};
            uint32_t nee_flags = 0, nee_light = 0;
            float light_sel_pdf = 1.f;
            if (valid) {
                float4 o4, d4;
                uint32_t fused_hidx = 0;
                const float4 h4 = B.hits[slot];
                if (bounce == 0 && P.gen_fused) {
                    const float4 cpf = B.beta[slot];
                    fused_hidx = f2b(cpf.z);
                    float cl0 = 0, cl1 = 0;
                    if (S.lens_radius > 0) {
                        cl0 = sample_dimension(S, s_perms, fused_hidx, 3);
                        cl1 = sample_dimension(S, s_perms, fused_hidx, 4);
                    }
                    F3 co, cd;
                    float ctm;
                    camera_ray<false>(S, cpf.x, cpf.y, cl0, cl1, &co, &cd, &ctm, opaque_zero());
                    o4 = make_float4(co.x, co.y, co.z, b2f(slot));
                    d4 = make_float4(cd.x, cd.y, cd.z, ctm);
                } else {
                    o4 = ro[slot];
                    d4 = rd[slot];
                }
                pid = f2b(o4.w);
                const float4 beta4 = bounce == 0 ? make_float4(1, 1, 1, 0) : rs[slot];
                const uint32_t state_w = bounce == 0 ? 5u : f2b(d4.w);
                beta = F3{beta4.x, beta4.y, beta4.z};
                dim = int(state_w & 0xffffu);
                const bool prev_specular = EXT && (state_w >> 16) != 0;
                hidx = bounce == 0 ? ((P.gen_fused) ? fused_hidx : B.hindex[pid]) : f2b(beta4.w);
                float u_nee[4] = {0, 0, 0, 0};
                if (bounce < S.max_depth) {
                    const int dim_u = __builtin_amdgcn_readfirstlane(dim);
                    sample_dimensions_n<4>(S, s_perms, dim_u + 1, __ballot(dim != dim_u) == 0, dim + 1, hidx, u_nee);
                }
                stamps.mark(1);
                const int prim = int(f2b(h4.x));
                const F3 ray_o = F3{o4.x, o4.y, o4.z};
                ray_d = F3{d4.x, d4.y, d4.z};
                float4 v0 = S.tri_verts[3 * size_t(prim)];
                float4 v1 = S.tri_verts[3 * size_t(prim) + 1];
                float4 v2 = S.tri_verts[3 * size_t(prim) + 2];
                keep_whole(v0, v1, v2);
                const uint32_t flags = f2b(v0.w);
                const int material = int(f2b(v1.w)), light = int(f2b(v2.w));
                if (flags & 1u) {
                    shape_hit_interaction<TEX, EXT>(S, S.prim_shape[prim], ray_o, ray_d, &is);
                } else {
                    triangle_interaction(S, prim, flags, F3{v0.x, v0.y, v0.z}, F3{v1.x, v1.y, v1.z},
                                         F3{v2.x, v2.y, v2.z}, ray_d, h4.y, h4.z, h4.w, &is);
                }
                if (EXT && S.probe_mode && bounce == 0) {
                    const F3 cv = is.p - ray_o;
                    const DProbeCam &cam = P.probe_cams[(pid / uint32_t(P.kc)) / (256u * uint32_t(P.probe_tiles))];
                    B.aux[pid] = make_float4(cam.nrm[0] * is.n.x + cam.nrm[1] * is.n.y + cam.nrm[2] * is.n.z,
                                             cam.nrm[3] * is.n.x + cam.nrm[4] * is.n.y + cam.nrm[5] * is.n.z,
                                             cam.nrm[6] * is.n.x + cam.nrm[7] * is.n.y + cam.nrm[8] * is.n.z, sqrtf(dot(cv, cv)));
                }
                if (((bounce == 0 && !(EXT && S.probe_mode)) || prev_specular) && light >= 0) {
                    const float4 L4 = B.L[pid];
                    const F3 L = F3{L4.x, L4.y, L4.z} + beta * area_light_L(S.lights[light], is.n, -ray_d);
                    B.L[pid] = make_float4(L.x, L.y, L.z, 0);
                }
                if (bounce < S.max_depth) {
                    surface = true;
                    if (TEX && S.textured_materials) {
                        const DMaterial &m0 = S.materials[material];
                        if (m0.kd_tex >= 0 || m0.ks_tex >= 0 || m0.kr_tex >= 0 || m0.kt_tex >= 0 || m0.bump_tex >= 0 || m0.rough_tex >= 0 || m0.sigma_tex >= 0 || m0.opacity_tex >= 0 || m0.rough_tex_v >= 0) {
                            TexDiff td = TexDiff{0, 0, 0, 0};
                            F3 dpdx = F3{0, 0, 0}, dpdy = F3{0, 0, 0};
                            if (bounce == 0) {
                                int px = 0, py = 0;
                                uint32_t kk = 0;
                                path_pixel(S, P, pid, &px, &py, &kk);
                                const float u0 = sample_dimension(S, s_perms, hidx, 0, px, py), u1 = sample_dimension(S, s_perms, hidx, 1, px, py);
                                float l0 = 0, l1 = 0;
                                if (S.lens_radius > 0) {
                                    l0 = sample_dimension(S, s_perms, hidx, 3);
                                    l1 = sample_dimension(S, s_perms, hidx, 4);
                                }
                                const RayDiff rdiff =
                                    S.probe_mode ? probe_differentials(S, P.probe_cams[(pid / uint32_t(P.kc)) / (256u * uint32_t(P.probe_tiles))],
                                                                       float(px) + u0, float(py) + u1, ray_o, ray_d)
                                                 : camera_differentials(S, float(px) + u0, float(py) + u1, l0, l1, ray_o, ray_d);
                                td = compute_differentials(is, rdiff, &dpdx, &dpdy);
                            }
                            if (m0.bump_tex >= 0) bump(S, m0.bump_tex, td, dpdx, dpdy, &is);
                            const DMaterial mm = textured_material(S, m0, is, td, dpdx, dpdy);
                            bsdf = make_bsdf<EXT>(mm, is);
                        } else {
                            bsdf = make_bsdf<EXT>(m0, is);
                        }
                    } else {
                        bsdf = make_bsdf<EXT>(S.materials[material], is);
                    }
                    stamps.mark(2);
                    if (n_nonspec(bsdf) > 0) {
                        ++n_nee;
                        int li = 0;
                        if (EXT && S.n_lights > 1) {
                            const float ul = sample_dimension_hi(S, s_perms, hidx, dim);
                            li = sample_light(S, is.p, ul, &light_sel_pdf);
                        }
                        if (S.n_lights > 0) ++dim;
                        if (S.n_lights > 0 && light_sel_pdf != 0) {
                            DLight lt_u;
                            DSphere lsp_u;
                            if (!EXT) {
                                lt_u = uniform_entry(S.lights, 0);
                                lsp_u = uniform_entry(S.spheres, lt_u.sphere);
                            }
                            const DLight &lt = EXT ? S.lights[li] : lt_u;
                            const DSphere &lsp = EXT ? S.spheres[lt.sphere] : lsp_u;
                            dim += 4;
                            nee_flags = estimate_direct_request<EXT, COUNT>(S, lt, &lsp, is, bsdf, u_nee[0], u_nee[1], u_nee[2], u_nee[3], so, sd,
                                                                            A, mo, md, Bc, &n_pdf_tests, &n_pdf_hits);
                            stamps.mark(3);
                            nee_light = uint32_t(li);
                            emit_nee = COUNT || nee_flags != 0;
                        }
                    }
                }
            }
            stamps.mark(4);
            const uint32_t eslot = out_take(nee_out, &B.counts[kCntNee + bounce], emit_nee, pad_nee);
            const bool emit_mis = emit_nee && (nee_flags & NEE_HAS_MIS) != 0;
            const uint32_t mslot = out_take(mis_out, &B.counts[kCntMis + bounce], emit_mis, pad_mis);
            if (emit_nee) {
                B.nee[eslot] = make_float4(so.x, so.y, so.z, light_sel_pdf);
                B.nee[plane + eslot] = make_float4(sd.x, sd.y, sd.z, b2f(nee_flags));
                if (nee_flags & NEE_HAS_MIS) {
                    B.nee[4 * plane + eslot] = make_float4(A.x, A.y, A.z, b2f(pid));
                    B.nee[5 * plane + eslot] = make_float4(Bc.x, Bc.y, Bc.z, b2f(nee_light));
                    B.nee[6 * plane + eslot] = make_float4(beta.x, beta.y, beta.z, b2f(pid));
                } else {
                    const F3 Ld = F3{0, 0, 0} + A;
                    const F3 pre = (__ballot(light_sel_pdf != 1.f) == 0) ? beta * Ld : beta * sdiv(Ld, light_sel_pdf);
                    B.nee[4 * plane + eslot] = make_float4(pre.x, pre.y, pre.z, b2f(pid));
                }
            }
            if (emit_mis) {
                B.nee[2 * plane + mslot] = make_float4(mo.x, mo.y, mo.z, b2f(eslot));
                B.nee[3 * plane + mslot] = make_float4(md.x, md.y, md.z, b2f(nee_light));
            }
        }
        stamps.mark(5);
        F3 next_o = F3{0, 0, 0}, next_d = F3{0, 0, 1};
        if (P.skip_last_bounce == 2 && bounce + 1 >= S.max_depth) surface = false;
        if (surface) {
            float u_bsdf[2];
            {
                const int dim_u = __builtin_amdgcn_readfirstlane(dim);
                sample_dimensions_n<2>(S, s_perms, dim_u, __ballot(dim != dim_u) == 0, dim, hidx, u_bsdf);
            }
            const float u0 = u_bsdf[0], u1 = u_bsdf[1];
            dim += 2;
            float pdf = 0;
            F3 wi = F3{0, 0, 0};
            bool sampled_specular = false, sampled_transmission = false;
            const F3 f = bsdf_sample_f(bsdf, -ray_d, &wi, u0, u1, &pdf, EXT, &sampled_specular, &sampled_transmission);
            float eta_scale = 1.f;
            if (EXT && S.has_glass && bounce > 0) eta_scale = B.eta_scale[pid];
            if (!(is_black(f) || pdf == 0.f)) {
                beta = beta * sdiv(f * absdot(wi, is.sn), pdf);
                const float by = lum_y(beta);
                if (by < 0.f || is_nan(by)) {
                    returned_early = true;
                } else {
                    next_o = offset_ray_origin(is.p, is.perr, is.n, wi);
                    next_d = wi;
                    alive = true;
                    if (sampled_specular && sampled_transmission) {
                        const float eta = bsdf.path_eta;
                        eta_scale *= (dot(-ray_d, is.n) > 0) ? (eta * eta) : 1 / (eta * eta);
                    }
                    const F3 rr_beta = beta * eta_scale;
                    const float mc = max3(rr_beta.x, rr_beta.y, rr_beta.z);
                    if (mc < S.rr_threshold && bounce > 3) {
                        const float q = mx(.05f, 1 - mc);
                        const float ur = sample_dimension_hi(S, s_perms, hidx, dim);
                        ++dim;
                        if (ur < q)
                            alive = false;
                        else
                            beta = sdiv(beta, 1 - q);
                    }
                }
            }
            if (EXT && P.skip_last_bounce == 1 && bounce + 1 >= S.max_depth && !sampled_specular) alive = false;
            if (EXT && alive && S.has_glass) B.eta_scale[pid] = eta_scale;
            state_next = uint32_t(dim) | (sampled_specular ? 0x10000u : 0u);
        }
        if (COUNT && valid && !alive && !returned_early) ++n_term;
        stamps.mark(6);
        const uint32_t nslot = out_take(ray_out, &B.counts[kCntRay + bounce + 1], alive, pad_ray);
        if (alive) {
            no[nslot] = make_float4(next_o.x, next_o.y, next_o.z, b2f(pid));
            nd[nslot] = make_float4(next_d.x, next_d.y, next_d.z, b2f(state_next));
            ns[nslot] = make_float4(beta.x, beta.y, beta.z, b2f(hidx));
        }
        stamps.mark(7);
      }
        __builtin_amdgcn_wave_barrier();
    }
    out_flush(ray_out, pad_ray);
    out_flush(nee_out, pad_nee);
    out_flush(mis_out, pad_mis);
    stamps.flush(B.counters, 0);
    if (COUNT) {
        flush_counter(&B.counters->nee_evals, n_nee);
        flush_counter(&B.counters->path_length[bounce < 7 ? bounce : 7], n_term);
        flush_counter(&B.counters->tri_tests, n_pdf_tests);
        flush_counter(&B.counters->tri_hits, n_pdf_hits);
    }
}


void launch_shade(const DScene &S, const PassDesc &P, const PassBuffers &B, int bounce, uint32_t max_rays, const LaunchCfg &cfg) {
    const bool tex_build = cfg.count_stats || S.textured_materials || S.probe_mode;
    const dim3 grid(grid_blocks(max_rays, cfg.n_cus, shade_waves(tex_build)));
    const size_t perm_bytes = S.sobol ? size_t(16) : (size_t(S.n_perms) * sizeof(uint16_t) + 15) & ~size_t(15);
    if (cfg.count_stats)
        hipLaunchKernelGGL((k_shade<true, true, true>), grid, dim3(kBlock), perm_bytes, cfg.stream, S, P, B, bounce, B.queue_cap);
    else
        if (S.textured_materials || S.probe_mode)
            hipLaunchKernelGGL((k_shade<false, true, true>), grid, dim3(kBlock), perm_bytes, cfg.stream, S, P, B, bounce, B.queue_cap);
        else if (S.extended_features)
            hipLaunchKernelGGL((k_shade<false, true, false>), grid, dim3(kBlock), perm_bytes, cfg.stream, S, P, B, bounce, B.queue_cap);
        else
            hipLaunchKernelGGL((k_shade<false, false, false>), grid, dim3(kBlock), perm_bytes, cfg.stream, S, P, B, bounce, B.queue_cap);
}
void launch_light_distributions(const DScene &S, const float *samples, float *out, const LaunchCfg &cfg) {
    const int n = S.light_nv[0] * S.light_nv[1] * S.light_nv[2];
    for (int l0 = 0; l0 < S.n_lights; l0 += 32768) {
        DScene part = S;
        part.lights = S.lights + l0;
        part.n_lights = std::min(S.n_lights - l0, 32768);
        hipLaunchKernelGGL(k_light_contrib, dim3((n + 127) / 128, part.n_lights), dim3(128), 0, cfg.stream, part, samples, out + l0,
                           light_record_floats(S.n_lights));
    }
    hipLaunchKernelGGL(k_light_cdf, dim3((n + 127) / 128), dim3(128), 0, cfg.stream, S, out);
}

}
```

pbrt-v3-iile_amd/csrc/device/kernels_trav.hip:

```cpp
#include "kcommon.h"

namespace iile {

template <bool COUNT, bool ALPHA, bool GEN>
__global__ __launch_bounds__(kTravBlock, IILE_TRAV_WAVES) void k_extend(DScene S, PassDesc P, PassBuffers B, int bounce) {
    const StackRef sr = trav_block_begin<COUNT, kTravBlock>(S, B.spill);
    const uint32_t count = B.counts[kCntRay + bounce];
    uint32_t *head = &B.counts[kCntExtHead + bounce];
    const float4 *ro = B.ray_o[bounce & 1], *rd = B.ray_d[bounce & 1];
    TraceStats st = {0, 0, 0, 0};
    unsigned long long n_rays = 0, n_term = 0;
    WaveFeed feed{0, 0, count == 0};
    WaveOut shade_out{0, 0};
    auto pad_shade = [&](uint32_t sl) { B.shade_q[sl] = kInvalid; };
    auto warm = [&](uint32_t first) {
        if (GEN) return;
        warm_plane(ro, first, count);
        warm_plane(rd, first, count);
    };
    Trav t;
    bool active = false;
    uint32_t slot = 0;
    float4 gen_d = make_float4(0, 0, 1, 0);
    DiagSums<IILE_SWITCH(IILE_TRAV_ITERSTATS) && !COUNT && !GEN, 8> iter_stat;
    DiagSums<IILE_SWITCH(IILE_TRAV_STAMPS) && !COUNT, 4> stamps;
    while (true) {
        stamps.mark(3);
        const unsigned long long idle_mask = __ballot(!active);
        if (refill_due(idle_mask, feed, GEN ? IILE_REFILL_IDLE_GEN : kRefillIdle, GEN ? IILE_REFILL_IDLE_GEN_SLOW : IILE_REFILL_IDLE_SLOW)) {
            uint32_t s_new;
            iter_stat.add(7, 1);
            if (feed_take(feed, head, count, !active, &s_new, warm)) {
                slot = s_new;
                if (GEN) {
                    const float z = opaque_zero();
                    B.L[slot] = make_float4(z, z, z, z);
                    int px = 0, py = 0;
                    uint32_t k = 0;
                    if (path_pixel(S, P, slot, &px, &py, &k)) {
                        const uint32_t idx = sample_index(S, px, py, k);
                        const float u0 = sample_dimension(S, idx, 0, px, py), u1 = sample_dimension(S, idx, 1, px, py);
                        float l0 = 0, l1 = 0;
                        if (S.lens_radius > 0) {
                            l0 = sample_dimension(S, idx, 3);
                            l1 = sample_dimension(S, idx, 4);
                        }
                        F3 o, d;
                        float tmax;
                        const float pfx = float(px) + u0, pfy = float(py) + u1;
                        flag_whole_film_position(B, slot, px, py, k, pfx, pfy, u0, u1);
                        camera_ray<false>(S, pfx, pfy, l0, l1, &o, &d, &tmax, opaque_zero());
                        B.beta[slot] = make_float4(pfx, pfy, b2f(idx), 0.f);
                        gen_d = make_float4(d.x, d.y, d.z, tmax);
                        trav_begin<COUNT>(S, t, o, d, tmax, &st, sr.root);
                        active = true;
                        ++n_rays;
                    }
                } else {
                    const float4 o4 = ro[slot], d4 = rd[slot];
                    if (f2b(o4.w) != kInvalid) {
                        trav_begin<COUNT>(S, t, F3{o4.x, o4.y, o4.z}, F3{d4.x, d4.y, d4.z}, bounce > 0 ? IILE_INF : d4.w, &st, sr.root);
                        active = true;
                        ++n_rays;
                        if (COUNT && B.nray_out) B.nray_out[2 * f2b(o4.w)] += 1;
                    }
                }
            }
        }
        stamps.mark(0);
        if (__ballot(active) == 0) {
            if (feed.exhausted) break;
            continue;
        }
        const WaveStep ws = trav_wave_step<COUNT, ALPHA, false>(S, active, t, sr, &st, false, GEN ? &gen_d : &rd[slot]);
        if (ws.kind >= 0) {
            iter_stat.add(3 * ws.kind, 1);
            iter_stat.add(3 * ws.kind + 1, uint32_t(ws.n_go));
            iter_stat.add(3 * ws.kind + 2, uint32_t(ws.n_wait));
            iter_stat.add(6, uint32_t(64 - ws.n_go - ws.n_wait));
            stamps.mark(1 + ws.kind);
        }
        const bool fin = active && !t.have;
        const bool is_hit = fin && t.hit_prim >= 0;
        if (fin) {
            if (is_hit || S.has_infinite) B.hits[slot] = make_float4(b2f(uint32_t(hit_index(t.hit_prim))), t.b0, t.b1, t.b2);
            active = false;
            if (COUNT && t.hit_prim < 0) ++n_term;
        }
        const uint32_t pos = out_take(shade_out, &B.counts[kCntShade + bounce], is_hit, pad_shade);
        if (is_hit) B.shade_q[pos] = slot | (uint32_t(t.hit_prim >> kHitClassShift) & 7u) << kSlotBits;
    }
    out_flush(shade_out, pad_shade);
    stamps.flush(B.counters, GEN ? 0 : 4);
    iter_stat.flush(B.counters, 0);
    flush_counter(&B.counters->ext_traced, n_rays);
    if (COUNT) {
        flush_counter(&B.counters->closest_rays, n_rays);
        flush_counter(&B.counters->ext_rays, n_rays);
        flush_counter(&B.counters->ext_nodes, st.nodes);
        flush_counter(&B.counters->ext_tri_tests, st.tris);
        flush_counter(&B.counters->ext_sphere_tests, st.spheres);
        flush_counter(&B.counters->nodes_closest, st.nodes);
        flush_counter(&B.counters->tri_tests, st.tris);
        flush_counter(&B.counters->tri_hits, st.tri_hits);
        flush_counter(&B.counters->sphere_tests, st.spheres);
        flush_counter(&B.counters->path_length[bounce < 7 ? bounce : 7], n_term);
    }
}



template <bool COUNT, bool ALPHA>
__global__ __launch_bounds__(kTravBlock, IILE_TRAV_WAVES) void k_shadow(DScene S, PassBuffers B, int bounce, uint32_t plane) {
    const StackRef sr = trav_block_begin<COUNT, kTravBlock>(S, B.spill);
    const uint32_t count = B.counts[kCntNee + bounce];
    uint32_t *head = &B.counts[kCntConHead + bounce];
    TraceStats st = {0, 0, 0, 0};
    unsigned long long n_shadow = 0, n_zero = 0;
    WaveFeed feed{0, 0, count == 0};
    Trav t;
    bool active = false, occluded = false;
    uint32_t e = 0, pid = 0;
    F3 L_old = F3{0, 0, 0}, add_unoccluded = F3{0, 0, 0}, add_occluded = F3{0, 0, 0};
    DiagSums<IILE_SWITCH(IILE_SHADOW_STAMPS) && !COUNT, 4> stamps;
    while (true) {
        stamps.mark(3);
        const unsigned long long idle_mask = __ballot(!active);
        if (refill_due(idle_mask, feed, kRefillIdle)) {
// ... 210 lines not shown
```

Before: 11660.

## Precompute Halton sample table per pixel class and read it in generate and shade kernels

Builds a device-side table at scene creation holding the camera, lens and per-bounce shading sample dimensions for every 128x128 pixel class and sample index. The generate, extend and shade kernels then load these values with a few float2/float4 reads instead of evaluating scrambled radical-inverse Halton dimensions per path. This trades per-sample arithmetic and permutation-table lookups for up to several GiB of extra device memory and bandwidth. The table is bypassed for stats, probe, list and out-of-range passes, and adds a new shade template variant.

```diff
diff --git a/include/iile_gpu.h b/include/iile_gpu.h
--- a/include/iile_gpu.h
+++ b/include/iile_gpu.h
@@ -74,6 +74,11 @@
                    int32_t *hit, iile_stats *stats);
 int iile_halton_samples(iile_scene *scene, int32_t n, const int32_t *px, const int32_t *py, const int32_t *k,
                         int32_t dim0, int32_t ndims, float *out, uint32_t *index_out);
+int iile_sample_table_records(iile_scene *scene, int32_t n, const int32_t *px, const int32_t *py, const int32_t *k, const int32_t *bounce,
+                              float *out8);
+uint64_t iile_sample_table_budget(void);
+void iile_test_sample_table_budget(uint64_t bytes);
+uint64_t iile_sample_table_bytes(const iile_scene *scene);
 int iile_camera_rays(iile_scene *scene, int32_t n, const float *pfilm2, const float *plens2, float *o3, float *d3);
 int iile_li_samples(iile_scene *scene, int32_t n, const int32_t *px, const int32_t *py, const int32_t *k,
                     float *L3, int32_t *nrays2);
diff --git a/pbrt-v3-iile_amd/binding.py b/pbrt-v3-iile_amd/binding.py
--- a/pbrt-v3-iile_amd/binding.py
+++ b/pbrt-v3-iile_amd/binding.py
@@ -197,7 +197,7 @@
 
 
 GPU_SYMBOLS = ["iile_device_count", "iile_last_error", "iile_scene_create", "iile_scene_destroy", "iile_render",
-               "iile_trace_closest", "iile_trace_any", "iile_shape_hit_attributes", "iile_halton_samples", "iile_camera_rays", "iile_li_samples",
+               "iile_trace_closest", "iile_trace_any", "iile_shape_hit_attributes", "iile_halton_samples", "iile_sample_table_records", "iile_sample_table_budget", "iile_test_sample_table_budget", "iile_sample_table_bytes", "iile_camera_rays", "iile_li_samples",
                "iile_bsdf_eval", "iile_bsdf_sample", "iile_bsdf_eval_ng", "iile_bsdf_sample_ng", "iile_bsdf_sample_specular", "iile_trig_probe", "iile_texture_eval", "iile_texture_eval_p", "iile_light_sample_li", "iile_light_sample_at", "iile_light_pdf_at", "iile_light_le", "iile_light_choose", "iile_render_probes",
                "iile_render_probes_reference", "iile_test_probe_ref_group", "iile_reference_points",
                "iile_device_select", "iile_device_alloc", "iile_device_free", "iile_device_download", "iile_device_upload", "iile_device_zero",
@@ -335,6 +335,12 @@
         lib.iile_traversal_limits.argtypes = [ctypes.POINTER(c_i32)]
         lib.iile_traversal_limits.restype = None
         lib.iile_test_patch_capacity.argtypes = [c_vp, c_u32]
+        lib.iile_sample_table_budget.argtypes = []
+        lib.iile_sample_table_budget.restype = c_u64
+        lib.iile_test_sample_table_budget.argtypes = [c_u64]
+        lib.iile_test_sample_table_budget.restype = None
+        lib.iile_sample_table_bytes.argtypes = [c_vp]
+        lib.iile_sample_table_bytes.restype = c_u64
         lib.iile_iispt_net_create.argtypes = [ctypes.POINTER(NetWeights), ctypes.POINTER(c_vp)]
         lib.iile_iispt_net_load.argtypes = [ctypes.c_char_p, ctypes.POINTER(c_vp)]
         lib.iile_iispt_net_forward.argtypes = [c_vp, c_vp, c_vp, c_i32, c_i32, c_vp, c_vp, c_i32]
@@ -604,6 +610,14 @@
             pass
 
 
+def sample_table_budget():
+    return int(gpu_lib().iile_sample_table_budget())
+
+
+def set_test_sample_table_budget(nbytes):
+    gpu_lib().iile_test_sample_table_budget(int(nbytes))
+
+
 class GpuScene:
 
     def __init__(self, host_scene):
@@ -632,7 +646,11 @@
             ptr = film.ctypes.data
         rc = gpu_lib().iile_render(self._s, ctypes.byref(prm), ptr, ctypes.byref(st) if want_stats else None)
         self._check(rc, "iile_render")
-        return film, (st.as_dict() if want_stats else None)
+        if not want_stats:
+            return film, None
+        d = st.as_dict()
+        d["sample_table_bytes"] = int(gpu_lib().iile_sample_table_bytes(self._s))
+        return film, d
 
     def render_status(self, stream=None):
         self._check(gpu_lib().iile_render_status(self._s, c_vp(stream) if stream else None), "iile_render_status")
@@ -679,6 +697,15 @@
         self._check(gpu_lib().iile_halton_samples(self._s, n, px.ctypes.data, py.ctypes.data, k.ctypes.data, dim0,
                                                   ndims, out.ctypes.data, idx.ctypes.data), "iile_halton_samples")
         return out, idx
+
+    def sample_table_records(self, px, py, k, bounce):
+        px, py, k, bounce = _i32(px), _i32(py), _i32(k), _i32(bounce)
+        out = np.empty((len(px), 8), np.float32)
+        f = gpu_lib().iile_sample_table_records
+        f.argtypes = [c_vp, c_i32, c_vp, c_vp, c_vp, c_vp, c_vp]
+        self._check(f(self._s, len(px), px.ctypes.data, py.ctypes.data, k.ctypes.data, bounce.ctypes.data, out.ctypes.data),
+                    "iile_sample_table_records")
+        return out
 
     def camera_rays(self, pfilm, plens=None):
         pfilm = _f32(pfilm)
diff --git a/pbrt-v3-iile_amd/csrc/device/api_common.h b/pbrt-v3-iile_amd/csrc/device/api_common.h
--- a/pbrt-v3-iile_amd/csrc/device/api_common.h
+++ b/pbrt-v3-iile_amd/csrc/device/api_common.h
@@ -109,6 +109,7 @@
     iile_probe_setup probe;
     const uint32_t *probe_pixel_offsets = nullptr;
     const float *probe_filter_table = nullptr;
+    uint64_t sample_table_bytes = 0;
     uint32_t *flag_count = nullptr;
     float *flag_rec = nullptr;
     iile::DevBlock probe_block;
@@ -137,6 +138,9 @@
 int ensure_film(iile_scene *sc, uint32_t n_tiles, uint32_t n_pixels, uint64_t n_wide = 0);
 int frame_pass(iile_scene *sc, const DScene &S, int rank, int nranks, hipStream_t stream, PassDesc *P);
 uint64_t path_budget(double bytes_per_path);
+constexpr uint64_t kSampleTableBudget = uint64_t(4) << 30;
+uint64_t sample_table_budget();
+void set_sample_table_budget(uint64_t bytes);
 int run_pass(iile_scene *sc, const DScene &S, int max_depth, const PassDesc &P_in, const LaunchCfg &cfg, bool timed, bool one_stream = false);
 void copy_counters(const DCounters &c, iile_stats *st);
 }
diff --git a/pbrt-v3-iile_amd/csrc/device/api_iispt.hip b/pbrt-v3-iile_amd/csrc/device/api_iispt.hip
--- a/pbrt-v3-iile_amd/csrc/device/api_iispt.hip
+++ b/pbrt-v3-iile_amd/csrc/device/api_iispt.hip
@@ -217,6 +217,7 @@
     S.filter_wide = 1;
     S.filter_table = sc->probe_filter_table;
     S.pixel_offsets = sc->probe_pixel_offsets;
+    clear_sample_table(&S);
     S.base_scale0 = pr.base_scales[0], S.base_scale1 = pr.base_scales[1];
     S.base_exp0 = pr.base_exponents[0], S.base_exp1 = pr.base_exponents[1];
     S.sample_stride = pr.sample_stride;
diff --git a/pbrt-v3-iile_amd/csrc/device/api_probes.hip b/pbrt-v3-iile_amd/csrc/device/api_probes.hip
--- a/pbrt-v3-iile_amd/csrc/device/api_probes.hip
+++ b/pbrt-v3-iile_amd/csrc/device/api_probes.hip
@@ -107,6 +107,25 @@
     if (index_out && (rc = dindex.get(index_out, n))) return rc;
     return IILE_OK;
 }
+
+int iile_sample_table_records(iile_scene *sc, int32_t n, const int32_t *px, const int32_t *py, const int32_t *k, const int32_t *bounce,
+                              float *out8) {
+    if (!sc || n < 0 || !px || !py || !k || !bounce || !out8) return api_fail(IILE_ERR_ARG, "iile_sample_table_records: bad argument");
+    if (!sc->ds.stab_shade) return api_fail(IILE_ERR_ARG, "iile_sample_table_records: the scene has no sample table");
+    for (int i = 0; i < n; ++i)
+        if (k[i] < 0 || uint32_t(k[i]) >= sc->ds.stab_spp || bounce[i] >= sc->ds.max_depth)
+            return api_fail(IILE_ERR_ARG, "iile_sample_table_records: sample or bounce outside the table");
+    int rc = ensure_device();
+    if (rc) return rc;
+    DevBuf<int> dx, dy, dk, db;
+    DevBuf<float> dout;
+    if ((rc = dx.put(px, n)) || (rc = dy.put(py, n)) || (rc = dk.put(k, n)) || (rc = db.put(bounce, n)) || (rc = dout.alloc(size_t(n) * 8))) return rc;
+    if (n) launch_sample_table_read(sc->ds, n, dx.p, dy.p, dk.p, db.p, dout.p, probe_cfg(sc));
+    return finish(dout, out8, size_t(n) * 8);
+}
+uint64_t iile_sample_table_budget(void) { return sample_table_budget(); }
+void iile_test_sample_table_budget(uint64_t bytes) { set_sample_table_budget(bytes); }
+uint64_t iile_sample_table_bytes(const iile_scene *sc) { return sc ? sc->sample_table_bytes : 0; }
 
 int iile_camera_rays(iile_scene *sc, int32_t n, const float *pfilm2, const float *plens2, float *o3, float *d3) {
     if (!sc || n < 0 || !pfilm2 || !o3 || !d3) return api_fail(IILE_ERR_ARG, "iile_camera_rays: bad argument");
diff --git a/pbrt-v3-iile_amd/csrc/device/api_render.hip b/pbrt-v3-iile_amd/csrc/device/api_render.hip
--- a/pbrt-v3-iile_amd/csrc/device/api_render.hip
+++ b/pbrt-v3-iile_amd/csrc/device/api_render.hip
@@ -241,9 +241,12 @@
     st->ext_rays_traced = c.ext_traced;
 }
 
-int run_pass(iile_scene *sc, const DScene &S, int max_depth, const PassDesc &P_in, const LaunchCfg &cfg, bool timed, bool one_stream) {
+int run_pass(iile_scene *sc, const DScene &S_in, int max_depth, const PassDesc &P_in, const LaunchCfg &cfg, bool timed, bool one_stream) {
     PassBuffers &B = sc->pb;
     PassDesc P = P_in;
+    DScene S = S_in;
+    if (cfg.count_stats || P.list_px || S.probe_mode || P.k0 < 0 || uint64_t(P.k0) + uint64_t(P.kc) > uint64_t(S.stab_spp) || max_depth > S.max_depth)
+        clear_sample_table(&S);
     P.gen_fused = !cfg.count_stats && !P.list_px && !S.has_infinite && !S.probe_mode && !B.nray_out && !S.env_camera;
     HIP_TRY(hipMemsetAsync(B.counts, 0, kCntWords * sizeof(uint32_t), cfg.stream));
     auto timed_launch_on = [&](hipStream_t stream, int kind, auto &&fn) -> int { return timed_step(sc, timed, stream, kind, fn); };
diff --git a/pbrt-v3-iile_amd/csrc/device/api_scene.hip b/pbrt-v3-iile_amd/csrc/device/api_scene.hip
--- a/pbrt-v3-iile_amd/csrc/device/api_scene.hip
+++ b/pbrt-v3-iile_amd/csrc/device/api_scene.hip
@@ -1,5 +1,8 @@
 #include <array>
+#include <chrono>
 #include <cmath>
+#include <cstdio>
+#include <cstdlib>
 #include <cstring>
 #include <limits>
 #include <map>
@@ -685,6 +688,60 @@
     return IILE_OK;
 }
 
+int build_sample_table(iile_scene *sc, const iile_scene_desc &d) {
+    DScene &S = sc->ds;
+    clear_sample_table(&S);
+    sc->sample_table_bytes = 0;
+    const int64_t spp = d.halton.spp;
+    if (S.sobol || S.max_depth <= 0 || spp <= 0 || S.sample_stride <= 0 || std::getenv("IILE_NO_SAMPLE_TABLE")) return IILE_OK;
+    if (5 + 7 * int64_t(S.max_depth) >= int64_t(S.n_hdims)) return IILE_OK;
+    const bool lens = S.lens_radius > 0;
+    const uint64_t per_slot = uint64_t(32) * uint64_t(S.max_depth) + (lens ? 16 : 8);
+    if (uint64_t(spp) > sample_table_budget() / (uint64_t(16384) * per_slot)) return IILE_OK;
+    const uint64_t slots = uint64_t(16384) * uint64_t(spp);
+    if (slots >= (uint64_t(1) << 32)) return IILE_OK;
+    const auto t0 = std::chrono::steady_clock::now();
+    S.stab_slots = uint32_t(slots), S.stab_spp = uint32_t(spp);
+    if (spp > 1) {
+        int l = 0;
+        while ((uint64_t(1) << l) < uint64_t(spp)) ++l;
+        S.stab_spp_magic = uint32_t((((uint64_t(1) << l) - uint64_t(spp)) << 32) / uint64_t(spp) + 1);
+        S.stab_spp_shift = uint32_t(l - 1);
+    }
+    float2 *cam = nullptr, *lens_part = nullptr;
+    float4 *shade = nullptr;
+    auto layout = [&](Carver c) {
+        cam = c.take<float2>(slots);
+        if (lens) lens_part = c.take<float2>(slots);
+        shade = c.take<float4>(slots * uint64_t(S.max_depth) * 2);
+        return c.used;
+    };
+    void *block = nullptr;
+    if (hipMalloc(&block, layout(Carver())) != hipSuccess) {
+        (void)hipGetLastError();
+        clear_sample_table(&S);
+        return IILE_OK;
+    }
+    sc->allocs.push_back(block);
+    layout(Carver(block));
+    launch_sample_table(S, cam, lens_part, shade, LaunchCfg{sc->n_cus, nullptr, false});
+    if (hipDeviceSynchronize() != hipSuccess || hipGetLastError() != hipSuccess) return api_fail(IILE_ERR_HIP, "sample table kernel failed");
+    S.stab_cam = cam, S.stab_lens = lens_part, S.stab_shade = shade;
+    sc->sample_table_bytes = slots * per_slot;
+    if (std::getenv("IILE_TIMING"))
+        fprintf(stderr, "iile timing: sample table of %.1f MiB built in %.3f s\n", double(sc->sample_table_bytes) / 1048576.0,
+                std::chrono::duration<double>(std::chrono::steady_clock::now() - t0).count());
+    return IILE_OK;
+}
+
+}
+
+namespace iile {
+namespace {
+uint64_t g_table_budget_override = 0;
+}
+uint64_t sample_table_budget() { return g_table_budget_override ? g_table_budget_override : kSampleTableBudget; }
+void set_sample_table_budget(uint64_t bytes) { g_table_budget_override = bytes; }
 }
 
 extern "C" {
@@ -783,7 +840,7 @@
         sc->n_cus = prop.multiProcessorCount;
     set_kernel_flags(*d, sc->ds);
     for (auto build : {build_bvh, build_top4, build_prims, build_shapes, build_materials, build_textures, build_lights, build_halton,
-                       build_sobol, build_camera_film, build_runtime, build_light_distribution}) {
+                       build_sobol, build_camera_film, build_runtime, build_light_distribution, build_sample_table}) {
         rc = build(sc, *d);
         if (rc) {
             iile_scene_destroy(sc);
diff --git a/pbrt-v3-iile_amd/csrc/device/dpath.h b/pbrt-v3-iile_amd/csrc/device/dpath.h
--- a/pbrt-v3-iile_amd/csrc/device/dpath.h
+++ b/pbrt-v3-iile_amd/csrc/device/dpath.h
@@ -153,6 +153,22 @@
     } else {
         for (int i = 0; i < N; ++i) out[i] = sample_dimension_hi(S, perms, index, dim_lane + i);
     }
+}
+
+DEV uint32_t sample_slot(const DScene &S, int px, int py, uint32_t k) {
+    int pmx = px - (px / 128) * 128, pmy = py - (py / 128) * 128;
+    if (pmx < 0) pmx += 128;
+    if (pmy < 0) pmy += 128;
+    return uint32_t(pmy * 128 + pmx) * S.stab_spp + k;
+}
+DEV uint32_t slot_halton_index(const DScene &S, uint32_t slot) {
+    const uint32_t cls = S.stab_spp > 1 ? div_magic(slot, S.stab_spp_magic, S.stab_spp_shift) : slot;
+    return S.pixel_offsets[cls] + (slot - cls * S.stab_spp) * uint32_t(S.sample_stride);
+}
+DEV void record_continuation(const float4 &ra, const float4 &rb, int off, float *u0, float *u1, float *ur) {
+    *u0 = off == 5 ? rb.y : (off == 1 ? ra.y : ra.x);
+    *u1 = off == 5 ? rb.z : (off == 1 ? ra.z : ra.y);
+    *ur = off == 5 ? rb.w : (off == 1 ? ra.w : ra.z);
 }
 
 DEV void concentric_sample_disk(float u0, float u1, float *dx, float *dy) {
diff --git a/pbrt-v3-iile_amd/csrc/device/dscene.h b/pbrt-v3-iile_amd/csrc/device/dscene.h
--- a/pbrt-v3-iile_amd/csrc/device/dscene.h
+++ b/pbrt-v3-iile_amd/csrc/device/dscene.h
@@ -155,6 +155,12 @@
     const float *filter_table;
     int base_scale0, base_scale1, base_exp0, base_exp1, sample_stride, mult_inv0, mult_inv1;
     int sample_center;
+    const float2 *stab_cam;
+    const float2 *stab_lens;
+    const float4 *stab_shade;
+    uint32_t stab_slots;
+    uint32_t stab_spp;
+    uint32_t stab_spp_magic, stab_spp_shift;
     int sobol, sobol_log2res, sobol_res, sobol_dims;
     const uint32_t *sobol_mat;
     const uint32_t *sobol_vdc;
@@ -163,6 +169,11 @@
     int max_depth;
     float rr_threshold;
 };
+inline void clear_sample_table(DScene *S) {
+    S->stab_cam = S->stab_lens = nullptr;
+    S->stab_shade = nullptr;
+    S->stab_slots = S->stab_spp = S->stab_spp_magic = S->stab_spp_shift = 0;
+}
 
 enum { NEE_HAS_SHADOW = 1, NEE_HAS_MIS = 2 };
 
diff --git a/pbrt-v3-iile_amd/csrc/device/kernels.h b/pbrt-v3-iile_amd/csrc/device/kernels.h
--- a/pbrt-v3-iile_amd/csrc/device/kernels.h
+++ b/pbrt-v3-iile_amd/csrc/device/kernels.h
@@ -95,6 +95,8 @@
 void launch_shadow(const DScene &S, const PassBuffers &B, int bounce, uint32_t max_rays, const LaunchCfg &cfg);
 void launch_mis(const DScene &S, const PassBuffers &B, int bounce, uint32_t max_rays, const LaunchCfg &cfg);
 void launch_light_distributions(const DScene &S, const float *samples, float *out, const LaunchCfg &cfg);
+void launch_sample_table(const DScene &S, float2 *cam, float2 *lens, float4 *shade, const LaunchCfg &cfg);
+void launch_sample_table_read(const DScene &S, int n, const int *px, const int *py, const int *k, const int *bounce, float *out, const LaunchCfg &cfg);
 void launch_miss(const DScene &S, const PassBuffers &B, int bounce, uint32_t max_rays, const LaunchCfg &cfg);
 void launch_mis_lit(const DScene &S, const PassBuffers &B, int bounce, uint32_t max_rays, const LaunchCfg &cfg);
 void launch_film_accumulate(const DScene &S, const PassDesc &P, const PassBuffers &B, const FilmBuffers &F,
diff --git a/pbrt-v3-iile_amd/csrc/device/kernels.hip b/pbrt-v3-iile_amd/csrc/device/kernels.hip
--- a/pbrt-v3-iile_amd/csrc/device/kernels.hip
+++ b/pbrt-v3-iile_amd/csrc/device/kernels.hip
@@ -13,12 +13,23 @@
         F3 o = F3{0, 0, 0}, d = F3{0, 0, 1};
         float tmax = 0;
         if (valid) {
-            const uint32_t idx = sample_index(S, px, py, k);
-            const float u0 = sample_dimension(S, idx, 0, px, py), u1 = sample_dimension(S, idx, 1, px, py);
-            float l0 = 0, l1 = 0;
-            if (S.lens_radius > 0) {
-                l0 = sample_dimension(S, idx, 3);
-                l1 = sample_dimension(S, idx, 4);
+            uint32_t idx;
+            float u0, u1, l0 = 0, l1 = 0;
+            if (S.stab_cam) {
+                idx = sample_slot(S, px, py, k);
+                const float2 cu = S.stab_cam[idx];
+                u0 = cu.x, u1 = cu.y;
+                if (S.lens_radius > 0) {
+                    const float2 cl = S.stab_lens[idx];
+                    l0 = cl.x, l1 = cl.y;
+                }
+            } else {
+                idx = sample_index(S, px, py, k);
+                u0 = sample_dimension(S, idx, 0, px, py), u1 = sample_dimension(S, idx, 1, px, py);
+                if (S.lens_radius > 0) {
+                    l0 = sample_dimension(S, idx, 3);
+                    l1 = sample_dimension(S, idx, 4);
+                }
             }
             if (P.probe_mode) {
                 const uint32_t probe = (pid / uint32_t(P.kc)) / (256u * uint32_t(P.probe_tiles));
diff --git a/pbrt-v3-iile_amd/csrc/device/kernels_shade.hip b/pbrt-v3-iile_amd/csrc/device/kernels_shade.hip
--- a/pbrt-v3-iile_amd/csrc/device/kernels_shade.hip
+++ b/pbrt-v3-iile_amd/csrc/device/kernels_shade.hip
@@ -1,4 +1,5 @@
 #include <cstdlib>
+#include <type_traits>
 
 #include "kcommon.h"
 
@@ -75,6 +76,39 @@
     }
 }
 
+__global__ __launch_bounds__(256) void k_sample_table(DScene S, float2 *cam, float2 *lens, float4 *shade) {
+    const uint32_t slot = blockIdx.x * blockDim.x + threadIdx.x;
+    if (slot >= S.stab_slots) return;
+    const uint32_t idx = slot_halton_index(S, slot);
+    if (blockIdx.y == 0) {
+        cam[slot] = make_float2(sample_dimension(S, idx, 0), sample_dimension(S, idx, 1));
+        if (lens) lens[slot] = make_float2(sample_dimension(S, idx, 3), sample_dimension(S, idx, 4));
+        return;
+    }
+    const int b = int(blockIdx.y) - 1, d0 = 5 + 7 * b;
+    float r[8];
+    for (int i = 0; i < 8; ++i) r[i] = sample_dimension_hi(S, S.perms, idx, d0 + i);
+    float4 *rec = shade + (size_t(b) * S.stab_slots + slot) * 2;
+    rec[0] = make_float4(r[0], r[1], r[2], r[3]);
+    rec[1] = make_float4(r[4], r[5], r[6], r[7]);
+}
+__global__ void k_sample_table_read(DScene S, int n, const int *px, const int *py, const int *k, const int *bounce, float *out) {
+    const int i = blockIdx.x * blockDim.x + threadIdx.x;
+    if (i >= n) return;
+    const uint32_t slot = sample_slot(S, px[i], py[i], uint32_t(k[i]));
+    float4 a = make_float4(0, 0, 0, 0), b = make_float4(0, 0, 0, 0);
+    if (bounce[i] < 0) {
+        const float2 c = S.stab_cam[slot];
+        a.x = c.x, a.y = c.y;
+        if (S.stab_lens) a.z = S.stab_lens[slot].x, a.w = S.stab_lens[slot].y;
+    } else {
+        const float4 *rec = S.stab_shade + (size_t(bounce[i]) * S.stab_slots + slot) * 2;
+        a = rec[0], b = rec[1];
+    }
+    reinterpret_cast<float4 *>(out)[2 * size_t(i)] = a;
+    reinterpret_cast<float4 *>(out)[2 * size_t(i) + 1] = b;
+}
+
 #ifndef IILE_SHADE_WAVES
 #define IILE_SHADE_WAVES 4
 #endif
@@ -82,15 +116,24 @@
 #define IILE_SHADE_WAVES_TEX 3
 #endif
 constexpr int shade_waves(bool tex) { return tex ? IILE_SHADE_WAVES_TEX : IILE_SHADE_WAVES; }
-template <bool COUNT, bool EXT, bool TEX>
+#ifndef IILE_SHADE_TAB_REREAD
+#define IILE_SHADE_TAB_REREAD 0
+#endif
+template <bool COUNT, bool EXT, bool TEX, bool TAB = false>
 __global__ __launch_bounds__(kBlock, shade_waves(TEX)) void k_shade(DScene S, PassDesc P, PassBuffers B, int bounce, uint32_t plane) {
-    extern __shared__ __attribute__((aligned(16))) uint16_t s_perms_raw[];
-    if (S.sobol) {
+    static_assert(!(TAB && COUNT), "the instrumented build keeps the digit chains");
+    typename std::conditional<TAB, const uint16_t *, lds_u16 *>::type s_perms;
+    if constexpr (TAB) {
+        s_perms = S.perms;
     } else {
-        for (int i = threadIdx.x; i < S.n_perms; i += kBlock) s_perms_raw[i] = S.perms[i];
-    }
-    __syncthreads();
-    lds_u16 *const s_perms = (lds_u16 *)s_perms_raw;
+        extern __shared__ __attribute__((aligned(16))) uint16_t s_perms_raw[];
+        if (S.sobol) {
+        } else {
+            for (int i = threadIdx.x; i < S.n_perms; i += kBlock) s_perms_raw[i] = S.perms[i];
+        }
+        __syncthreads();
+        s_perms = (lds_u16 *)s_perms_raw;
+    }
     const uint32_t count = B.counts[kCntShade + bounce];
     const float4 *ro = B.ray_o[bounce & 1], *rd = B.ray_d[bounce & 1];
     float4 *no = B.ray_o[(bounce + 1) & 1], *nd = B.ray_d[(bounce + 1) & 1];
@@ -139,6 +182,9 @@
         bool alive = false, returned_early = false;
         uint32_t pid = 0, hidx = 0;
         int dim = 0;
+        bool tab_wave = false;
+        float4 rec_a = make_float4(0, 0, 0, 0), rec_b = make_float4(0, 0, 0, 0);
+        auto chain_index = [&]() { return TAB ? slot_halton_index(S, hidx) : hidx; };
         Isect is;
         Bsdf bsdf;
         F3 beta = F3{0, 0, 0}, ray_d = F3{0, 0, 1};
@@ -158,8 +204,13 @@
                     fused_hidx = f2b(cpf.z);
                     float cl0 = 0, cl1 = 0;
                     if (S.lens_radius > 0) {
-                        cl0 = sample_dimension(S, s_perms, fused_hidx, 3);
-                        cl1 = sample_dimension(S, s_perms, fused_hidx, 4);
+                        if (TAB) {
+                            const float2 cl = S.stab_lens[fused_hidx];
+                            cl0 = cl.x, cl1 = cl.y;
+                        } else {
+                            cl0 = sample_dimension(S, s_perms, fused_hidx, 3);
+                            cl1 = sample_dimension(S, s_perms, fused_hidx, 4);
+                        }
                     }
                     F3 co, cd;
                     float ctm;
@@ -180,7 +231,20 @@
                 float u_nee[4] = {0, 0, 0, 0};
                 if (bounce < S.max_depth) {
                     const int dim_u = __builtin_amdgcn_readfirstlane(dim);
-                    sample_dimensions_n<4>(S, s_perms, dim_u + 1, __ballot(dim != dim_u) == 0, dim + 1, hidx, u_nee);
+                    const bool dim_uniform = __ballot(dim != dim_u) == 0;
+                    if (TAB) {
+                        tab_wave = dim_uniform && dim_u == 5 + 7 * bounce;
+                        if (tab_wave) {
+                            const float4 *rec = S.stab_shade + (size_t(bounce) * S.stab_slots + hidx) * 2;
+                            rec_a = rec[0];
+                            rec_b = rec[1];
+                            u_nee[0] = rec_a.y, u_nee[1] = rec_a.z, u_nee[2] = rec_a.w, u_nee[3] = rec_b.x;
+                        } else {
+                            sample_dimensions_n<4>(S, s_perms, dim_u + 1, false, dim + 1, chain_index(), u_nee);
+                        }
+                    } else {
+                        sample_dimensions_n<4>(S, s_perms, dim_u + 1, dim_uniform, dim + 1, hidx, u_nee);
+                    }
                 }
                 stamps.mark(1);
                 const int prim = int(f2b(h4.x));
@@ -221,11 +285,20 @@
                                 int px = 0, py = 0;
                                 uint32_t kk = 0;
                                 path_pixel(S, P, pid, &px, &py, &kk);
-                                const float u0 = sample_dimension(S, s_perms, hidx, 0, px, py), u1 = sample_dimension(S, s_perms, hidx, 1, px, py);
-                                float l0 = 0, l1 = 0;
-                                if (S.lens_radius > 0) {
-                                    l0 = sample_dimension(S, s_perms, hidx, 3);
-                                    l1 = sample_dimension(S, s_perms, hidx, 4);
+                                float u0, u1, l0 = 0, l1 = 0;
+                                if (TAB) {
+                                    const float2 cu = S.stab_cam[hidx];
+                                    u0 = cu.x, u1 = cu.y;
+                                    if (S.lens_radius > 0) {
+                                        const float2 cl = S.stab_lens[hidx];
+                                        l0 = cl.x, l1 = cl.y;
+                                    }
+                                } else {
+                                    u0 = sample_dimension(S, s_perms, hidx, 0, px, py), u1 = sample_dimension(S, s_perms, hidx, 1, px, py);
+                                    if (S.lens_radius > 0) {
+                                        l0 = sample_dimension(S, s_perms, hidx, 3);
+                                        l1 = sample_dimension(S, s_perms, hidx, 4);
+                                    }
                                 }
                                 const RayDiff rdiff =
                                     S.probe_mode ? probe_differentials(S, P.probe_cams[(pid / uint32_t(P.kc)) / (256u * uint32_t(P.probe_tiles))],
@@ -247,7 +320,11 @@
                         ++n_nee;
                         int li = 0;
                         if (EXT && S.n_lights > 1) {
-                            const float ul = sample_dimension_hi(S, s_perms, hidx, dim);
+                            float ul;
+                            if (TAB && tab_wave)
+                                ul = rec_a.x;
+                            else
+                                ul = sample_dimension_hi(S, s_perms, chain_index(), dim);
                             li = sample_light(S, is.p, ul, &light_sel_pdf);
                         }
                         if (S.n_lights > 0) ++dim;
@@ -296,10 +373,19 @@
         F3 next_o = F3{0, 0, 0}, next_d = F3{0, 0, 1};
         if (P.skip_last_bounce == 2 && bounce + 1 >= S.max_depth) surface = false;
         if (surface) {
-            float u_bsdf[2];
-            {
+            float u_bsdf[2], ur_tab = 0;
+            if (TAB && tab_wave) {
+                const int off = dim - (5 + 7 * bounce);
+                if (IILE_SHADE_TAB_REREAD) {
+                    const float *rf = reinterpret_cast<const float *>(S.stab_shade + (size_t(bounce) * S.stab_slots + hidx) * 2) + off;
+                    u_bsdf[0] = rf[0], u_bsdf[1] = rf[1];
+                    if (bounce > 3) ur_tab = rf[2];
+                } else {
+                    record_continuation(rec_a, rec_b, off, &u_bsdf[0], &u_bsdf[1], &ur_tab);
+                }
+            } else {
                 const int dim_u = __builtin_amdgcn_readfirstlane(dim);
-                sample_dimensions_n<2>(S, s_perms, dim_u, __ballot(dim != dim_u) == 0, dim, hidx, u_bsdf);
+                sample_dimensions_n<2>(S, s_perms, dim_u, !TAB && __ballot(dim != dim_u) == 0, dim, chain_index(), u_bsdf);
             }
             const float u0 = u_bsdf[0], u1 = u_bsdf[1];
             dim += 2;
@@ -326,7 +412,11 @@
                     const float mc = max3(rr_beta.x, rr_beta.y, rr_beta.z);
                     if (mc < S.rr_threshold && bounce > 3) {
                         const float q = mx(.05f, 1 - mc);
-                        const float ur = sample_dimension_hi(S, s_perms, hidx, dim);
+                        float ur;
+                        if (TAB && tab_wave)
+                            ur = ur_tab;
+                        else
+                            ur = sample_dimension_hi(S, s_perms, chain_index(), dim);
                         ++dim;
                         if (ur < q)
                             alive = false;
@@ -368,7 +458,14 @@
     const bool tex_build = cfg.count_stats || S.textured_materials || S.probe_mode;
     const dim3 grid(grid_blocks(max_rays, cfg.n_cus, shade_waves(tex_build)));
     const size_t perm_bytes = S.sobol ? size_t(16) : (size_t(S.n_perms) * sizeof(uint16_t) + 15) & ~size_t(15);
-    if (cfg.count_stats)
+    if (S.stab_shade && !cfg.count_stats) {
+        if (S.textured_materials)
+            hipLaunchKernelGGL((k_shade<false, true, true, true>), grid, dim3(kBlock), 0, cfg.stream, S, P, B, bounce, B.queue_cap);
+        else if (S.extended_features)
+            hipLaunchKernelGGL((k_shade<false, true, false, true>), grid, dim3(kBlock), 0, cfg.stream, S, P, B, bounce, B.queue_cap);
+        else
+            hipLaunchKernelGGL((k_shade<false, false, false, true>), grid, dim3(kBlock), 0, cfg.stream, S, P, B, bounce, B.queue_cap);
+    } else if (cfg.count_stats)
         hipLaunchKernelGGL((k_shade<true, true, true>), grid, dim3(kBlock), perm_bytes, cfg.stream, S, P, B, bounce, B.queue_cap);
     else
         if (S.textured_materials || S.probe_mode)
@@ -378,6 +475,12 @@
         else
             hipLaunchKernelGGL((k_shade<false, false, false>), grid, dim3(kBlock), perm_bytes, cfg.stream, S, P, B, bounce, B.queue_cap);
 }
+void launch_sample_table(const DScene &S, float2 *cam, float2 *lens, float4 *shade, const LaunchCfg &cfg) {
+    hipLaunchKernelGGL(k_sample_table, dim3((S.stab_slots + 255) / 256, 1 + S.max_depth), dim3(256), 0, cfg.stream, S, cam, lens, shade);
+}
+void launch_sample_table_read(const DScene &S, int n, const int *px, const int *py, const int *k, const int *bounce, float *out, const LaunchCfg &cfg) {
+    hipLaunchKernelGGL(k_sample_table_read, dim3((n + 127) / 128), dim3(128), 0, cfg.stream, S, n, px, py, k, bounce, out);
+}
 void launch_light_distributions(const DScene &S, const float *samples, float *out, const LaunchCfg &cfg) {
     const int n = S.light_nv[0] * S.light_nv[1] * S.light_nv[2];
     for (int l0 = 0; l0 < S.n_lights; l0 += 32768) {
diff --git a/pbrt-v3-iile_amd/csrc/device/kernels_trav.hip b/pbrt-v3-iile_amd/csrc/device/kernels_trav.hip
--- a/pbrt-v3-iile_amd/csrc/device/kernels_trav.hip
+++ b/pbrt-v3-iile_amd/csrc/device/kernels_trav.hip
@@ -38,12 +38,23 @@
                     int px = 0, py = 0;
                     uint32_t k = 0;
                     if (path_pixel(S, P, slot, &px, &py, &k)) {
-                        const uint32_t idx = sample_index(S, px, py, k);
-                        const float u0 = sample_dimension(S, idx, 0, px, py), u1 = sample_dimension(S, idx, 1, px, py);
-                        float l0 = 0, l1 = 0;
-                        if (S.lens_radius > 0) {
-                            l0 = sample_dimension(S, idx, 3);
-                            l1 = sample_dimension(S, idx, 4);
+                        uint32_t idx;
+                        float u0, u1, l0 = 0, l1 = 0;
+                        if (S.stab_cam) {
+                            idx = sample_slot(S, px, py, k);
+                            const float2 cu = S.stab_cam[idx];
+                            u0 = cu.x, u1 = cu.y;
+                            if (S.lens_radius > 0) {
+                                const float2 cl = S.stab_lens[idx];
+                                l0 = cl.x, l1 = cl.y;
+                            }
+                        } else {
+                            idx = sample_index(S, px, py, k);
+                            u0 = sample_dimension(S, idx, 0, px, py), u1 = sample_dimension(S, idx, 1, px, py);
+                            if (S.lens_radius > 0) {
+                                l0 = sample_dimension(S, idx, 3);
+                                l1 = sample_dimension(S, idx, 4);
+                            }
                         }
                         F3 o, d;
                         float tmax;
```

Result: faster. 12000 (median of 6 runs) (+2.9%).
